# Chris10M/Lip2Speech

Hardware: AMD Instinct MI355X
Metric: mel-frames/sec at LRW batch=32, 29-frame clips (Lip2Speech.inference, S=300) (higher is better)
Workload: dtype f32; 1 GPU; LRW single-word, batch=32 per step, 29x96x96 RGB mouth crops, S=300 decode steps, speaker embedding supplied (encoding=voice), random-init weights; every step is one full pass over one B=32 batch; frames=29, decode_steps=300, library=libl2s_hip.so, parallelism=dp1 (clip sharding, no collective), batches_per_launch_chain=8, launch_chains_in_flight_per_gpu=3, distinct_batches_per_gpu=24, ranks=1

## Files before the change

### lip2speech_amd/csrc/encoder_kernels.hip

```cpp
#include "l2s_common.h"
#include <type_traits>

namespace l2s {

constexpr int FE_PR = 6;
constexpr int FE_CR = 2 * FE_PR + 1;
constexpr int FE_XROWS = 2 * (FE_CR - 1) + 7 + 1;
constexpr int FE_XLD = 104;
constexpr int FE_KP = 50;
constexpr int FE_CO = 24;

template <int HW, int MODE>
__global__ __launch_bounds__(256, 3) void frontend3d_kernel(const FrontendW w, const FrameSrc vsrc,
                                                            int T, float* __restrict__ out, float* __restrict__ zout) {
    constexpr bool SAVE_Z = MODE == 1;
    constexpr int H = HW, W = HW, Hc = H / 2, Wc = W / 2, Hp = Hc / 2, Wp = Wc / 2;
    constexpr int P = FE_CR * Wc;
    constexpr int NT = (P + 31) / 32;
    constexpr int TPW = (NT + 3) / 4;
    constexpr int XS = FE_XROWS * FE_XLD;
    constexpr int WS = FE_KP * 32;
    constexpr int CS = MODE == 2 ? 0 : P * (FE_CO / 2);
    constexpr int SMEM = (XS + WS) > CS ? (XS + WS) : CS;
    __shared__ __attribute__((aligned(16))) float smem[SMEM];
// ... 44 lines not shown
#pragma unroll
        for (int s = 0; s < FE_KP / 2; ++s) {
            const int k0 = 2 * s, k1 = 2 * s + 1;
            const int off0 = (k0 / 7) * FE_XLD + (k0 % 7);
            const int off1 = (k1 / 7) * FE_XLD + (k1 % 7);
            const int off = lg ? off1 : off0;
            const float bw = Ws[(2 * s + lg) * 32 + li];
#pragma unroll
            for (int j = 0; j < TPW; ++j) {
                if (wave + 4 * j < NT) {
                    const float a = Xs[base[j] + off];
                    acc[j] = __builtin_amdgcn_mfma_f32_32x32x2f32(a, bw, acc[j], 0, 0, 0);
                }
            }
        }
    }
    __syncthreads();

    if (MODE == 2) {
        float s1 = 0.f, s2 = 0.f;
#pragma unroll
        for (int j = 0; j < TPW; ++j) {
            if (wave + 4 * j < NT) {
#pragma unroll
                for (int r = 0; r < 16; ++r) {
                    const int p = (wave + 4 * j) * 32 + (r & 3) + 8 * (r >> 2) + 4 * lg;
                    const int lr = p / Wc, crow = 2 * p0 - 1 + lr;
                    if (p < P && lr >= 1 && crow < Hc) {
                        s1 += acc[j][r]; s2 = fmaf(acc[j][r], acc[j][r], s2);
                        if (out && li < FE_CO) out[(((int64_t)f * Hc + crow) * Wc + (p - lr * Wc)) * FE_CO + li] = acc[j][r];
                    }
                }
            }
        }
        float* red = smem;
        red[((0 * 4 + wave) * 2 + lg) * 32 + li] = s1;
        red[((1 * 4 + wave) * 2 + lg) * 32 + li] = s2;
        __syncthreads();
        if (tid < 2 * FE_CO) {
            const int k = tid / FE_CO, ch = tid - k * FE_CO;
            float t = 0.f;
            for (int q = 0; q < 8; ++q) t += red[(k * 8 + q) * 32 + ch];
            zout[((int64_t)(blockIdx.y * gridDim.x + blockIdx.x) * 2 + k) * FE_CO + ch] = t;
        }
        return;
    }
    float* Cs = smem;
    constexpr int CH = FE_CO / 2;
    const float sc = li < FE_CO ? w.scale[li] : 0.f, sh = li < FE_CO ? w.shift[li] : 0.f, sl = li < FE_CO ? w.slope[li] : 0.f;
#pragma unroll
    for (int half = 0; half < 2; ++half) {
        if (li >= half * CH && li < (half + 1) * CH) {
#pragma unroll
            for (int j = 0; j < TPW; ++j) {
                if (wave + 4 * j < NT) {
#pragma unroll
                    for (int r = 0; r < 16; ++r) {
                        const int p = (wave + 4 * j) * 32 + (r & 3) + 8 * (r >> 2) + 4 * lg;
                        if (p < P) {
                            float v = acc[j][r] * sc + sh;
                            if (SAVE_Z) {
                                const int lr = p / Wc, crow = 2 * p0 - 1 + lr;
                                if (lr >= 1 && crow < Hc) zout[(((int64_t)f * Hc + crow) * Wc + (p - lr * Wc)) * FE_CO + li] = v;
                            }
                            v = v >= 0.f ? v : sl * v;
                            Cs[p * CH + (li - half * CH)] = v;
                        }
                    }
                }
            }
        }
        __syncthreads();
        for (int i = tid; i < FE_PR * Wp * CH; i += 256) {
            const int ch = i % CH;
            const int pw = (i / CH) % Wp;
            const int prl = i / (CH * Wp);
            const int pr = p0 + prl;
            if (pr >= Hp) continue;
            float m = -INFINITY;
#pragma unroll
            for (int dr = 0; dr < 3; ++dr) {
                const int crow = 2 * pr - 1 + dr;
                if (crow < 0 || crow >= Hc) continue;
                const int lrow = 2 * prl + dr;
#pragma unroll
                for (int dc = -1; dc <= 1; ++dc) {
                    const int cc = 2 * pw + dc;
                    if (cc < 0 || cc >= Wc) continue;
                    m = fmaxf(m, Cs[(lrow * Wc + cc) * CH + ch]);
                }
            }
            out[(((int64_t)f * Hp + pr) * Wp + pw) * FE_CO + half * CH + ch] = m;
        }
        __syncthreads();
    }
}

template <int HW> struct FxGeom { static constexpr int XLD = HW == 96 ? 112 : 108, PLANE = FE_XROWS * XLD * 2; };
constexpr int FX_WROW = 48;

typedef __bf16 fx_bf16x8 __attribute__((ext_vector_type(8)));

__device__ __forceinline__ void fx_split4(const float4& v, uint2& hi, uint2& mid, uint2& lo) {
    const float f[4] = {v.x, v.y, v.z, v.w};
    unsigned h[4], m[4], l[4];
#pragma unroll
    for (int e = 0; e < 4; ++e) {
        const unsigned xb = __float_as_uint(f[e]);
        const float r1 = f[e] - __uint_as_float(xb & 0xFFFF0000u);
        const float r2 = r1 - __uint_as_float(__float_as_uint(r1) & 0xFFFF0000u);
        h[e] = xb; m[e] = __float_as_uint(r1); l[e] = __float_as_uint(r2);
    }
    hi = make_uint2(__builtin_amdgcn_perm(h[1], h[0], 0x07060302u), __builtin_amdgcn_perm(h[3], h[2], 0x07060302u));
    mid = make_uint2(__builtin_amdgcn_perm(m[1], m[0], 0x07060302u), __builtin_amdgcn_perm(m[3], m[2], 0x07060302u));
    lo = make_uint2(__builtin_amdgcn_perm(l[1], l[0], 0x07060302u), __builtin_amdgcn_perm(l[3], l[2], 0x07060302u));
}

typedef __bf16 fx_bf16x2 __attribute__((ext_vector_type(2)));
__device__ __forceinline__ unsigned fx_rne2(float a, float b) { fx_bf16x2 v = {(__bf16)a, (__bf16)b}; return __builtin_bit_cast(unsigned, v); }

template <int HW, int TERMS>
__global__ __launch_bounds__(256, 3) void frontend3d_x3_kernel(const FrontendW w, const FrameSrc vsrc, int T, float* __restrict__ out) {
    constexpr int FX_WSLAB = 4 * TERMS * 32 * FX_WROW;
    constexpr int H = HW, W = HW, Hc = H / 2, Wc = W / 2, Hp = Hc / 2, Wp = Wc / 2;
    constexpr int P = FE_CR * Wc;
    constexpr int NT = (P + 31) / 32;
    constexpr int TPW = (NT + 3) / 4;
    constexpr int XLD = FxGeom<HW>::XLD, PLANE = FxGeom<HW>::PLANE;
    static_assert((2 * (XLD / 2)) % 32 == Wc % 32 && XLD >= W + 8, "row pitch: conflict-free straddling tiles");
    constexpr int XS = TERMS * PLANE;
    constexpr int CS = P * (FE_CO / 2) * 4;
    constexpr int SMEM = (XS + FX_WSLAB) > CS ? (XS + FX_WSLAB) : CS;
    constexpr int NLD = ((FE_XROWS - 1) * (W / 4) + 255) / 256;
    constexpr int NWL = (FX_WSLAB / 16 + 255) / 256;
    __shared__ __attribute__((aligned(16))) unsigned char smem[SMEM];
    unsigned char* const Xs = smem;
    unsigned char* const Ws = smem + XS;

    const int f = blockIdx.y;
    const int bg = f / T, t = f - bg * T;
    const int grp = bg / vsrc.per, b = bg - grp * vsrc.per;
    const float* __restrict__ video = vsrc.p[grp];
    const int p0 = blockIdx.x * FE_PR;
    const int tid = threadIdx.x, wave = tid >> 6, lane = tid & 63;
    const int li = lane & 31, lg = lane >> 5;

    for (int i = tid; i < XS / 16; i += 256) reinterpret_cast<uint4*>(Xs)[i] = make_uint4(0u, 0u, 0u, 0u);

    int base[TPW];
#pragma unroll
    for (int j = 0; j < TPW; ++j) {
        int p = (wave + 4 * j) * 32 + li;
        p = p < P ? p : P - 1;
        const int lr = p / Wc, c = p - lr * Wc;
        base[j] = ((2 * lr + lg) * XLD + 2 * c) * 2;
    }
    f32x16 acc[TPW];
#pragma unroll
    for (int j = 0; j < TPW; ++j)
#pragma unroll
        for (int r = 0; r < 16; ++r) acc[j][r] = 0.f;

    const int gy0 = 4 * p0 - 5;
    auto valid = [&](int slab) { const int tt = t + (slab % 5) - 2; return tt >= 0 && tt < T; };
    auto next_valid = [&](int slab) { while (slab < 15 && !valid(slab)) ++slab; return slab; };

    float4 rin[NLD];
    uint4 rw[NWL];
    auto fetch = [&](int slab) {
        const int ci = slab / 5, kt = slab - ci * 5;
        const float* src = video + ((int64_t)(b * 3 + ci) * T + (t + kt - 2)) * (H * W);
#pragma unroll
        for (int q = 0; q < NLD; ++q) {
            const int i = tid + 256 * q;
            const int row = i / (W / 4), x4 = i - row * (W / 4);
            const int gy = gy0 + row;
            rin[q] = make_float4(0.f, 0.f, 0.f, 0.f);
            if (i < (FE_XROWS - 1) * (W / 4) && gy >= 0 && gy < H) rin[q] = *reinterpret_cast<const float4*>(src + gy * W + 4 * x4);
        }
        const uint4* wsrc = reinterpret_cast<const uint4*>(TERMS == 3 ? w.w3 : w.w1) + (int64_t)slab * (FX_WSLAB / 16);
#pragma unroll
        for (int q = 0; q < NWL; ++q) {
            const int i = tid + 256 * q;
            rw[q] = i < FX_WSLAB / 16 ? wsrc[i] : make_uint4(0u, 0u, 0u, 0u);
        }
    };
    auto stage = [&]() {
#pragma unroll
        for (int q = 0; q < NLD; ++q) {
            const int i = tid + 256 * q;
            if (i < (FE_XROWS - 1) * (W / 4)) {
                const int row = i / (W / 4), x4 = i - row * (W / 4);
                unsigned char* d = Xs + (row * XLD + 4 + 4 * x4) * 2;
                if constexpr (TERMS == 3) {
                    uint2 hi, mid, lo;
                    fx_split4(rin[q], hi, mid, lo);
                    *reinterpret_cast<uint2*>(d) = hi; *reinterpret_cast<uint2*>(d + PLANE) = mid; *reinterpret_cast<uint2*>(d + 2 * PLANE) = lo;
                } else {
                    *reinterpret_cast<uint2*>(d) = make_uint2(fx_rne2(rin[q].x, rin[q].y), fx_rne2(rin[q].z, rin[q].w));
                }
            }
        }
#pragma unroll
        for (int q = 0; q < NWL; ++q) {
            const int i = tid + 256 * q;
            if (i < FX_WSLAB / 16) reinterpret_cast<uint4*>(Ws)[i] = rw[q];
        }
    };

    int slab = next_valid(0);
    if (slab < 15) fetch(slab);
    while (slab < 15) {
        __syncthreads();
        stage();
        const int nxt = next_valid(slab + 1);
        if (nxt < 15) fetch(nxt);
        __syncthreads();
#pragma unroll
        for (int s = 0; s < 4; ++s) {
            const unsigned char* wp = Ws + ((s * TERMS) * 32 + li) * FX_WROW + lg * 16;
            const fx_bf16x8 bh = *reinterpret_cast<const fx_bf16x8*>(wp);
            if constexpr (TERMS == 1) {
#pragma unroll
                for (int j = 0; j < TPW; ++j) {
                    if (wave + 4 * j < NT) {
                        const unsigned* ap = reinterpret_cast<const unsigned*>(Xs + base[j] + s * (2 * XLD * 2));
                        const fx_bf16x8 ah = __builtin_bit_cast(fx_bf16x8, make_uint4(ap[0], ap[1], ap[2], ap[3]));
                        acc[j] = __builtin_amdgcn_mfma_f32_32x32x16_bf16(ah, bh, acc[j], 0, 0, 0);
                    }
                }
            } else {
            const fx_bf16x8 bm = *reinterpret_cast<const fx_bf16x8*>(wp + 32 * FX_WROW);
            const fx_bf16x8 bl = *reinterpret_cast<const fx_bf16x8*>(wp + 64 * FX_WROW);
#pragma unroll
            for (int j = 0; j < TPW; ++j) {
                if (wave + 4 * j < NT) {
                    const unsigned* ap = reinterpret_cast<const unsigned*>(Xs + base[j] + s * (2 * XLD * 2));
                    const unsigned* am_ = reinterpret_cast<const unsigned*>(Xs + base[j] + s * (2 * XLD * 2) + PLANE);
                    const unsigned* al_ = reinterpret_cast<const unsigned*>(Xs + base[j] + s * (2 * XLD * 2) + 2 * PLANE);
                    const fx_bf16x8 ah = __builtin_bit_cast(fx_bf16x8, make_uint4(ap[0], ap[1], ap[2], ap[3]));
                    const fx_bf16x8 am = __builtin_bit_cast(fx_bf16x8, make_uint4(am_[0], am_[1], am_[2], am_[3]));
                    const fx_bf16x8 al = __builtin_bit_cast(fx_bf16x8, make_uint4(al_[0], al_[1], al_[2], al_[3]));
                    acc[j] = __builtin_amdgcn_mfma_f32_32x32x16_bf16(al, bh, acc[j], 0, 0, 0);
                    acc[j] = __builtin_amdgcn_mfma_f32_32x32x16_bf16(ah, bl, acc[j], 0, 0, 0);
                    acc[j] = __builtin_amdgcn_mfma_f32_32x32x16_bf16(am, bm, acc[j], 0, 0, 0);
                    acc[j] = __builtin_amdgcn_mfma_f32_32x32x16_bf16(am, bh, acc[j], 0, 0, 0);
                    acc[j] = __builtin_amdgcn_mfma_f32_32x32x16_bf16(ah, bm, acc[j], 0, 0, 0);
                    acc[j] = __builtin_amdgcn_mfma_f32_32x32x16_bf16(ah, bh, acc[j], 0, 0, 0);
                }
            }
            }
        }
        slab = nxt;
    }
    __syncthreads();

    float* Cs = reinterpret_cast<float*>(smem);
    constexpr int CH = FE_CO / 2;
    const float sc = li < FE_CO ? w.scale[li] : 0.f, sh = li < FE_CO ? w.shift[li] : 0.f, sl = li < FE_CO ? w.slope[li] : 0.f;
#pragma unroll
    for (int half = 0; half < 2; ++half) {
        if (li >= half * CH && li < (half + 1) * CH) {
#pragma unroll
            for (int j = 0; j < TPW; ++j) {
                if (wave + 4 * j < NT) {
#pragma unroll
                    for (int r = 0; r < 16; ++r) {
                        const int p = (wave + 4 * j) * 32 + (r & 3) + 8 * (r >> 2) + 4 * lg;
                        if (p < P) {
                            float v = acc[j][r] * sc + sh;
                            v = v >= 0.f ? v : sl * v;
                            Cs[p * CH + (li - half * CH)] = v;
                        }
                    }
                }
            }
        }
        __syncthreads();
        for (int i = tid; i < FE_PR * Wp * CH; i += 256) {
            const int ch = i % CH;
            const int pw = (i / CH) % Wp;
            const int prl = i / (CH * Wp);
            const int pr = p0 + prl;
            if (pr >= Hp) continue;
            float m = -INFINITY;
#pragma unroll
            for (int dr = 0; dr < 3; ++dr) {
                const int crow = 2 * pr - 1 + dr;
                if (crow < 0 || crow >= Hc) continue;
                const int lrow = 2 * prl + dr;
#pragma unroll
                for (int dc = -1; dc <= 1; ++dc) {
                    const int cc = 2 * pw + dc;
                    if (cc < 0 || cc >= Wc) continue;
                    m = fmaxf(m, Cs[(lrow * Wc + cc) * CH + ch]);
                }
            }
            out[(((int64_t)f * Hp + pr) * Wp + pw) * FE_CO + half * CH + ch] = m;
        }
        __syncthreads();
    }
}

template <int HW>
__global__ __launch_bounds__(256, 2) void frontend3d_x3p_kernel(const FrontendW w, const FrameSrc vsrc, int T, float* __restrict__ out) {
    constexpr int H = HW, W = HW, Hc = H / 2, Wc = W / 2, Hp = Hc / 2, Wp = Wc / 2;
    constexpr int P = FE_CR * Wc;
    constexpr int PT = (P + 15) / 16;
    constexpr int TPW = (PT + 3) / 4;
    constexpr int XLD = 112, PLANE = FE_XROWS * XLD * 2;
    static_assert(XLD >= W + 8 && (XLD / 2) % 32 == 24, "row pitch");
    constexpr int XS = 3 * PLANE;
    constexpr int WROW = 48, LROW = 32;
    constexpr int WSP = 24 * LROW;
    constexpr int WSO = 12 * WSP;
    constexpr int WS = 2 * WSO;
    constexpr int CS = P * (FE_CO / 2) * 4;
    constexpr int SMEM = (XS + 2 * WS) > CS ? (XS + 2 * WS) : CS;
    constexpr int NLD = ((FE_XROWS - 1) * (W / 4) + 255) / 256;
    constexpr int NWU = WS / 16, NWC = NWU / 64;
    static_assert(NWU % 64 == 0, "the weight operand is a whole number of wave-wide 16-byte pieces");
    constexpr int SRC_SP = 32 * WROW / 16;
    __shared__ __attribute__((aligned(16))) unsigned char smem[SMEM];
    unsigned char* const Xs = smem;
    unsigned char* const Ws0 = smem + XS;

    const int NPAIR = (T + 1) / 2;
    const int bg = blockIdx.y / NPAIR, t0 = 2 * (blockIdx.y - bg * NPAIR);
    const bool has1 = t0 + 1 < T;
    const int grp = bg / vsrc.per, b = bg - grp * vsrc.per;
    const float* __restrict__ video = vsrc.p[grp];
    const int p0 = blockIdx.x * FE_PR;
    const int tid = threadIdx.x, wave = tid >> 6, lane = tid & 63;
    const int li = lane & 15, kg = lane >> 4;
    const int kr = ((kg & 1) << 1) | (kg >> 1);

    for (int i = tid; i < XS / 16; i += 256) reinterpret_cast<uint4*>(Xs)[i] = make_uint4(0u, 0u, 0u, 0u);

    int base[TPW];
#pragma unroll
    for (int j = 0; j < TPW; ++j) {
        int p = (wave + 4 * j) * 16 + li;
        p = p < P ? p : P - 1;
        const int lr = p / Wc, c = p - lr * Wc;
        base[j] = ((2 * lr + kr) * XLD + 2 * c) * 2;
    }
    int wof[3];
#pragma unroll
    for (int nt = 0; nt < 3; ++nt) {
        const int q = nt * 16 + li, o = q >= FE_CO ? 1 : 0, ch = q - FE_CO * o;
        wof[nt] = o * WSO + (kr >> 1) * (3 * WSP) + ch * LROW + (kr & 1) * 16;
    }
    f32x4 acc[TPW][3];
#pragma unroll
    for (int j = 0; j < TPW; ++j)
#pragma unroll
        for (int nt = 0; nt < 3; ++nt) acc[j][nt] = {0.f, 0.f, 0.f, 0.f};

    const int gy0 = 4 * p0 - 5;
    auto valid = [&](int sl) { const int d = sl % 6, tau = t0 - 2 + d; return tau >= 0 && tau < T && (d <= 4 || has1); };
    auto next_valid = [&](int sl) { while (sl < 18 && !valid(sl)) ++sl; return sl; };

    float4 rin[NLD];
    auto fetch_piece = [&](int sl, int q) {
        const int ci = sl / 6, d = sl - ci * 6;
        const float* src = video + ((int64_t)(b * 3 + ci) * T + (t0 - 2 + d)) * (H * W);
        const int i = tid + 256 * q;
        const int row = i / (W / 4), x4 = i - row * (W / 4);
        const int gy = gy0 + row;
        rin[q] = make_float4(0.f, 0.f, 0.f, 0.f);
        if (i < (FE_XROWS - 1) * (W / 4) && gy >= 0 && gy < H) rin[q] = *reinterpret_cast<const float4*>(src + gy * W + 4 * x4);
    };
    auto fetch = [&](int sl) {
#pragma unroll
        for (int q = 0; q < NLD; ++q) fetch_piece(sl, q);
    };
    auto dma_piece = [&](int sl, int buf, int kp) {
        const int c = wave + 4 * kp;
        if (c < NWC) {
            const int ci = sl / 6, d = sl - ci * 6;
            const uint4* w3 = reinterpret_cast<const uint4*>(w.w3);
            unsigned char* const Wd = Ws0 + buf * WS;
            const int i = c * 64 + lane;
            const int o = i >= NWU / 2 ? 1 : 0, r = i - o * (NWU / 2);
            const int sp = r / (WSP / 16), u = r - sp * (WSP / 16);
            const int kt = d - o;
            const bool on = kt >= 0 && kt <= 4 && (o == 0 || has1);
            const uint4* src = on ? w3 + (int64_t)(ci * 5 + kt) * (12 * SRC_SP) + sp * SRC_SP + (u >> 1) * (WROW / 16) + (u & 1) : w3 + (24 * WROW) / 16;
            __builtin_amdgcn_global_load_lds((const __attribute__((address_space(1))) void*)src,
                                             (__attribute__((address_space(3))) void*)(Wd + c * 1024), 16, 0, 0);
        }
    };
    constexpr int NDP = (NWC + 3) / 4;
    auto dma_weights = [&](int sl, int buf) {
#pragma unroll
        for (int kp = 0; kp < NDP; ++kp) dma_piece(sl, buf, kp);
    };
    auto stage = [&]() {
#pragma unroll
        for (int q = 0; q < NLD; ++q) {
            const int i = tid + 256 * q;
            if (i < (FE_XROWS - 1) * (W / 4)) {
                const int row = i / (W / 4), x4 = i - row * (W / 4);
                unsigned char* dd = Xs + (row * XLD + 4 + 4 * x4) * 2;
                uint2 hi, mid, lo;
                fx_split4(rin[q], hi, mid, lo);
                *reinterpret_cast<uint2*>(dd) = hi; *reinterpret_cast<uint2*>(dd + PLANE) = mid; *reinterpret_cast<uint2*>(dd + 2 * PLANE) = lo;
            }
        }
    };

    int sl = next_valid(0), nslab = 0;
    if (sl < 18) { fetch(sl); dma_weights(sl, 0); }
    while (sl < 18) {
        __syncthreads();
        stage();
        const int d = sl % 6;
        const bool on0 = d <= 4, on1 = d >= 1 && has1;
        const int nxt = next_valid(sl + 1);
        __syncthreads();
        const bool more = nxt < 18;
        static_assert(NDP + NLD <= 2 * TPW, "one request per pixel tile");
        const unsigned char* const Ws = Ws0 + (nslab & 1) * WS;
#pragma unroll
        for (int S = 0; S < 2; ++S) {
            fx_bf16x8 bh[3], bm[3], bl[3];
#pragma unroll
            for (int nt = 0; nt < 3; ++nt) {
                const unsigned char* wp = Ws + wof[nt] + S * (2 * 3 * WSP);
                bh[nt] = *reinterpret_cast<const fx_bf16x8*>(wp);
                bm[nt] = *reinterpret_cast<const fx_bf16x8*>(wp + WSP);
                bl[nt] = *reinterpret_cast<const fx_bf16x8*>(wp + 2 * WSP);
            }
#pragma unroll
            for (int j = 0; j < TPW; ++j) {
                if (more) {
                    const int pos = S * TPW + j;
                    if (pos < NDP) dma_piece(nxt, (nslab + 1) & 1, pos);
                    else if (pos < NDP + NLD) fetch_piece(nxt, pos - NDP);
                }
                {
                    const unsigned* ap = reinterpret_cast<const unsigned*>(Xs + base[j] + S * (4 * XLD * 2));
                    const unsigned* am_ = reinterpret_cast<const unsigned*>(Xs + base[j] + S * (4 * XLD * 2) + PLANE);
                    const unsigned* al_ = reinterpret_cast<const unsigned*>(Xs + base[j] + S * (4 * XLD * 2) + 2 * PLANE);
                    const fx_bf16x8 ah = __builtin_bit_cast(fx_bf16x8, make_uint4(ap[0], ap[1], ap[2], ap[3]));
                    const fx_bf16x8 am = __builtin_bit_cast(fx_bf16x8, make_uint4(am_[0], am_[1], am_[2], am_[3]));
                    const fx_bf16x8 al = __builtin_bit_cast(fx_bf16x8, make_uint4(al_[0], al_[1], al_[2], al_[3]));
#pragma unroll
                    for (int nt = 0; nt < 3; ++nt) {
                        if ((nt == 0 && !on0) || (nt == 2 && !on1)) continue;
                        f32x4 a = acc[j][nt];
                        a = __builtin_amdgcn_mfma_f32_16x16x32_bf16(al, bh[nt], a, 0, 0, 0);
                        a = __builtin_amdgcn_mfma_f32_16x16x32_bf16(ah, bl[nt], a, 0, 0, 0);
                        a = __builtin_amdgcn_mfma_f32_16x16x32_bf16(am, bm[nt], a, 0, 0, 0);
                        a = __builtin_amdgcn_mfma_f32_16x16x32_bf16(am, bh[nt], a, 0, 0, 0);
                        a = __builtin_amdgcn_mfma_f32_16x16x32_bf16(ah, bm[nt], a, 0, 0, 0);
                        a = __builtin_amdgcn_mfma_f32_16x16x32_bf16(ah, bh[nt], a, 0, 0, 0);
                        acc[j][nt] = a;
                    }
                }
            }
        }
        sl = nxt; ++nslab;
    }
    __syncthreads();

    float* Cs = reinterpret_cast<float*>(smem);
    constexpr int CH = FE_CO / 2;
    float sc[3], sh[3], slp[3];
#pragma unroll
    for (int nt = 0; nt < 3; ++nt) {
        const int q = nt * 16 + li, ch = q >= FE_CO ? q - FE_CO : q;
        sc[nt] = w.scale[ch]; sh[nt] = w.shift[ch]; slp[nt] = w.slope[ch];
    }
    for (int pass = 0; pass < (has1 ? 4 : 2); ++pass) {
        const int o = pass >> 1, half = pass & 1;
#pragma unroll
        for (int nt = 0; nt < 3; ++nt) {
            const int q = nt * 16 + li, qo = q >= FE_CO ? 1 : 0, ch = q - FE_CO * qo;
            if (qo == o && ch >= half * CH && ch < (half + 1) * CH) {
#pragma unroll
                for (int j = 0; j < TPW; ++j) {
                    if (wave + 4 * j < PT) {
#pragma unroll
                        for (int r = 0; r < 4; ++r) {
                            const int p = (wave + 4 * j) * 16 + 4 * kg + r;
                            if (p < P) {
                                float v = acc[j][nt][r] * sc[nt] + sh[nt];
                                v = v >= 0.f ? v : slp[nt] * v;
                                Cs[p * CH + (ch - half * CH)] = v;
                            }
                        }
                    }
                }
            }
        }
        __syncthreads();
        const int f = bg * T + t0 + o;
        for (int i = tid; i < FE_PR * Wp * CH; i += 256) {
            const int ch = i % CH;
            const int pw = (i / CH) % Wp;
            const int prl = i / (CH * Wp);
            const int pr = p0 + prl;
            if (pr >= Hp) continue;
            float m = -INFINITY;
#pragma unroll
            for (int dr = 0; dr < 3; ++dr) {
                const int crow = 2 * pr - 1 + dr;
                if (crow < 0 || crow >= Hc) continue;
                const int lrow = 2 * prl + dr;
#pragma unroll
                for (int dc = -1; dc <= 1; ++dc) {
                    const int cc = 2 * pw + dc;
                    if (cc < 0 || cc >= Wc) continue;
                    m = fmaxf(m, Cs[(lrow * Wc + cc) * CH + ch]);
                }
            }
            out[(((int64_t)f * Hp + pr) * Wp + pw) * FE_CO + half * CH + ch] = m;
        }
        __syncthreads();
    }
}

template <int HW>
__global__ __launch_bounds__(256, 2) void frontend3d_x3q_kernel(const FrontendW w, const FrameSrc vsrc, int T, float* __restrict__ out) {
    const int NPAIR = (T + 1) / 2;
    const int bg = blockIdx.y / NPAIR, t0 = 2 * (blockIdx.y - bg * NPAIR);
    const bool has1 = t0 + 1 < T;
    const int grp = bg / vsrc.per, b = bg - grp * vsrc.per;
    const float* __restrict__ video = vsrc.p[grp];
#define FE_X3Q_PITCH T
#define FE_X3Q_FRAME0 (bg * T)
#include "frontend_x3q_block.inc"
#undef FE_X3Q_PITCH
#undef FE_X3Q_FRAME0
}

template <int HW>
__global__ __launch_bounds__(256, 2) void frontend3d_x3q_ragged_kernel(const FrontendW w, const FrameSrc vsrc, const RaggedClip* __restrict__ clips,
                                                                       const int* __restrict__ pair_clip, float* __restrict__ out) {
    const RaggedClip k = clips[pair_clip[blockIdx.y]];
    const int T = k.len;
    const int t0 = 2 * ((int)blockIdx.y - k.pair0);
    const bool has1 = t0 + 1 < T;
    const int b = k.row;
    const float* __restrict__ video = vsrc.p[0];
#pragma unroll
    for (int g = 1; g < MAX_GROUP; ++g) video = k.g == g ? vsrc.p[g] : video;
#define FE_X3Q_PITCH k.T
#define FE_X3Q_FRAME0 k.frame0
#include "frontend_x3q_block.inc"
#undef FE_X3Q_PITCH
#undef FE_X3Q_FRAME0
}

int launch_frontend(const FrontendW& w, const FrameSrc& video, int B, int T, int H, int W, float* out, hipStream_t s, float* zout) {
    L2S_REQUIRE(H == W && (H == 96 || H == 88), "frontend supports 96x96 and 88x88 mouth crops");
    L2S_REQUIRE(video.per >= 1 && (B + video.per - 1) / video.per <= MAX_GROUP, "too many frame tensors in one launch");
    for (int g = 0; g < (B + video.per - 1) / video.per; ++g)
        L2S_REQUIRE(video.p[g] && (reinterpret_cast<uintptr_t>(video.p[g]) & 15u) == 0, "video must be non-null and 16-byte aligned");
    const int Hp = H / 4;
    dim3 grid((Hp + FE_PR - 1) / FE_PR, B * T);
    ProfScope ps("frontend3d_conv_bn_prelu_pool", s);
    if (!zout && w.w1) {
        if (H == 96) hipLaunchKernelGGL((frontend3d_x3_kernel<96, 1>), grid, dim3(256), 0, s, w, video, T, out);
        else hipLaunchKernelGGL((frontend3d_x3_kernel<88, 1>), grid, dim3(256), 0, s, w, video, T, out);
    } else if (!zout && w.w3 && w.pair) {
        dim3 gp((Hp + FE_PR - 1) / FE_PR, B * ((T + 1) / 2));
        if (w.pipe) {
            const unsigned pad = w.solo ? 4096u : 0u;
            if (H == 96) hipLaunchKernelGGL((frontend3d_x3q_kernel<96>), gp, dim3(256), pad, s, w, video, T, out);
            else hipLaunchKernelGGL((frontend3d_x3q_kernel<88>), gp, dim3(256), pad, s, w, video, T, out);
        } else if (H == 96) hipLaunchKernelGGL((frontend3d_x3p_kernel<96>), gp, dim3(256), 0, s, w, video, T, out);
        else hipLaunchKernelGGL((frontend3d_x3p_kernel<88>), gp, dim3(256), 0, s, w, video, T, out);
    } else if (!zout && w.w3) {
        if (H == 96) hipLaunchKernelGGL((frontend3d_x3_kernel<96, 3>), grid, dim3(256), 0, s, w, video, T, out);
        else hipLaunchKernelGGL((frontend3d_x3_kernel<88, 3>), grid, dim3(256), 0, s, w, video, T, out);
    } else if (zout) {
        if (H == 96) hipLaunchKernelGGL((frontend3d_kernel<96, 1>), grid, dim3(256), 0, s, w, video, T, out, zout);
        else hipLaunchKernelGGL((frontend3d_kernel<88, 1>), grid, dim3(256), 0, s, w, video, T, out, zout);
    } else {
        if (H == 96) hipLaunchKernelGGL((frontend3d_kernel<96, 0>), grid, dim3(256), 0, s, w, video, T, out, zout);
        else hipLaunchKernelGGL((frontend3d_kernel<88, 0>), grid, dim3(256), 0, s, w, video, T, out, zout);
    }
    L2S_CHECK_HIP(hipGetLastError());
    return 0;
}

int launch_frontend_ragged(const FrontendW& w, const FrameSrc& video, const RaggedTab& rg, int H, int W, float* out, hipStream_t s) {
    L2S_REQUIRE(H == W && (H == 96 || H == 88), "frontend supports 96x96 and 88x88 mouth crops");
    L2S_REQUIRE(w.w3 && !w.w1 && w.pair && w.pipe && !w.solo, "the ragged front-end exists in the default form only (frontend_x3 = 3, no infer_bf16)");
    L2S_REQUIRE(rg.clips && rg.pair_clip && rg.NP >= 1 && rg.NF >= 1, "ragged front-end: empty table");
    const int Hp = H / 4;
    dim3 gp((Hp + FE_PR - 1) / FE_PR, rg.NP);
    prof_count("frontend3d_ragged_pair_blocks", rg.NP);
    ProfScope ps("frontend3d_conv_bn_prelu_pool_ragged", s);
    if (H == 96) hipLaunchKernelGGL((frontend3d_x3q_ragged_kernel<96>), gp, dim3(256), 0, s, w, video, rg.clips, rg.pair_clip, out);
    else hipLaunchKernelGGL((frontend3d_x3q_ragged_kernel<88>), gp, dim3(256), 0, s, w, video, rg.clips, rg.pair_clip, out);
    L2S_CHECK_HIP(hipGetLastError());
    return 0;
}

__global__ __launch_bounds__(256) void frontend_pool_kernel(const float* __restrict__ z, const float* __restrict__ slope, int NF, int Hc, int Wc, float* __restrict__ out) {
    const int Hp = Hc / 2, Wp = Wc / 2;
    const unsigned total = (unsigned)NF * Hp * Wp * FE_CO;
    for (unsigned idx = blockIdx.x * 256u + threadIdx.x; idx < total; idx += gridDim.x * 256u) {
        const int ch = idx % FE_CO;
        unsigned r = idx / FE_CO;
        const int pw = r % Wp; r /= Wp;
        const int pr = r % Hp;
        const unsigned f = r / Hp;
        const float sl = slope[ch];
        float m = -INFINITY;
#pragma unroll
        for (int dr = -1; dr <= 1; ++dr) {
            const int crow = 2 * pr + dr;
            if (crow < 0 || crow >= Hc) continue;
#pragma unroll
            for (int dc = -1; dc <= 1; ++dc) {
                const int cc = 2 * pw + dc;
                if (cc < 0 || cc >= Wc) continue;
                float v = z[((size_t)(f * Hc + crow) * Wc + cc) * FE_CO + ch];
                v = v >= 0.f ? v : sl * v;
                m = fmaxf(m, v);
            }
        }
        out[idx] = m;
    }
}
int launch_frontend_pool(const float* z, const float* slope, int NF, int Hc, int Wc, float* out, hipStream_t s) {
    const int64_t total = (int64_t)NF * (Hc / 2) * (Wc / 2) * FE_CO;
    L2S_REQUIRE(total < (int64_t)1 << 31, "front-end pool: map too large for 32-bit indexing");
    ProfScope ps("train_frontend_prelu_pool", s);
    hipLaunchKernelGGL(frontend_pool_kernel, dim3((unsigned)std::min<int64_t>((total + 255) / 256, 16384)), dim3(256), 0, s, z, slope, NF, Hc, Wc, out);
    L2S_CHECK_HIP(hipGetLastError());
    return 0;
}

int launch_frontend_stats(const FrontendW& w, const float* video1, int B, int T, int H, int W, float* partials, int* nblocks, hipStream_t s, float* raw_out) {
    L2S_REQUIRE(H == W && (H == 96 || H == 88), "frontend supports 96x96 and 88x88 mouth crops");
    FrameSrc video{}; video.p[0] = video1; video.per = B;
    const int Hp = H / 4;
    dim3 grid((Hp + FE_PR - 1) / FE_PR, B * T);
    *nblocks = (int)(grid.x * grid.y);
    ProfScope ps("train_frontend3d_stats", s);
    if (H == 96) hipLaunchKernelGGL((frontend3d_kernel<96, 2>), grid, dim3(256), 0, s, w, video, T, raw_out, partials);
    else hipLaunchKernelGGL((frontend3d_kernel<88, 2>), grid, dim3(256), 0, s, w, video, T, raw_out, partials);
    L2S_CHECK_HIP(hipGetLastError());
    return 0;
}

struct ClipTab { int64_t off[MAX_COLLATE_CLIPS]; int frames[MAX_COLLATE_CLIPS]; };

__global__ __launch_bounds__(256) void normalise_pad_kernel(const uint8_t* __restrict__ packed, const ClipTab tab, int b0, int T, int HW4,
                                                            float* __restrict__ video) {
    const int q = blockIdx.x * 256 + threadIdx.x, t = blockIdx.y, bl = blockIdx.z;
    if (q >= HW4) return;
    const int b = b0 + bl;
    const int64_t plane = (int64_t)HW4 * 4;
    float* out = video + (((int64_t)b * 3) * T + t) * plane + (int64_t)q * 4;
    float4 r = make_float4(0.f, 0.f, 0.f, 0.f), g = r, bl4 = r;
    if (t < tab.frames[bl]) {
        const uint32_t* src = reinterpret_cast<const uint32_t*>(packed + tab.off[bl] + ((int64_t)t * plane + (int64_t)q * 4) * 3);
        const uint32_t w0 = src[0], w1 = src[1], w2 = src[2];
        const float mean[3] = {0.485f, 0.456f, 0.406f}, stdv[3] = {0.229f, 0.224f, 0.225f};
        auto nrm = [&](uint32_t byte, int c) { return __fdiv_rn(__fsub_rn(__fdiv_rn((float)byte, 255.0f), mean[c]), stdv[c]); };
        r = make_float4(nrm(w0 & 255u, 0), nrm(w0 >> 24, 0), nrm((w1 >> 16) & 255u, 0), nrm((w2 >> 8) & 255u, 0));
        g = make_float4(nrm((w0 >> 8) & 255u, 1), nrm(w1 & 255u, 1), nrm(w1 >> 24, 1), nrm((w2 >> 16) & 255u, 1));
        bl4 = make_float4(nrm((w0 >> 16) & 255u, 2), nrm((w1 >> 8) & 255u, 2), nrm(w2 & 255u, 2), nrm(w2 >> 24, 2));
    }
    *reinterpret_cast<float4*>(out) = r;
    *reinterpret_cast<float4*>(out + (int64_t)T * plane) = g;
    *reinterpret_cast<float4*>(out + 2 * (int64_t)T * plane) = bl4;
}

int launch_normalise_pad(const uint8_t* packed, const int64_t* offsets, const int* frames, int B, int T, int H, int W, float* video, hipStream_t s) {
    L2S_REQUIRE((H * W) % 4 == 0 && (reinterpret_cast<uintptr_t>(packed) & 3u) == 0 && (reinterpret_cast<uintptr_t>(video) & 15u) == 0,
                "frames: H*W must be a multiple of 4, buffers aligned");
    const int HW4 = H * W / 4;
    ProfScope ps("normalise_pad_frames", s);
    for (int b0 = 0; b0 < B; b0 += MAX_COLLATE_CLIPS) {
        const int nb = B - b0 < MAX_COLLATE_CLIPS ? B - b0 : MAX_COLLATE_CLIPS;
        ClipTab tab{};
        for (int i = 0; i < nb; ++i) {
            L2S_REQUIRE(frames[b0 + i] >= 0 && frames[b0 + i] <= T && offsets[b0 + i] % 4 == 0, "clip table: 0 <= frames <= T, 4-byte aligned offsets");
            tab.off[i] = offsets[b0 + i]; tab.frames[i] = frames[b0 + i];
        }
        hipLaunchKernelGGL(normalise_pad_kernel, dim3((HW4 + 255) / 256, T, nb), dim3(256), 0, s, packed, tab, b0, T, HW4, video);
    }
    L2S_CHECK_HIP(hipGetLastError());
    return 0;
}

__global__ __launch_bounds__(256) void dwconv3x3_kernel(const float* __restrict__ in, int N, int Hi, int Wi, int ldi,
                                                        int ci_off, int C, int stride, const float* __restrict__ w9,
                                                        const float* __restrict__ scale, const float* __restrict__ shift,
                                                        float* __restrict__ out, int Ho, int Wo, int ldo, int co_off) {
    const int64_t total = (int64_t)N * Ho * Wo * C;
    for (int64_t idx = (int64_t)blockIdx.x * 256 + threadIdx.x; idx < total; idx += (int64_t)gridDim.x * 256) {
        const int c = idx % C;
        int64_t r = idx / C;
        const int ow = r % Wo;
        r /= Wo;
        const int oh = r % Ho;
        const int n = r / Ho;
        float acc = 0.f;
#pragma unroll
        for (int kh = 0; kh < 3; ++kh) {
            const int ih = oh * stride + kh - 1;
            if (ih < 0 || ih >= Hi) continue;
#pragma unroll
            for (int kw = 0; kw < 3; ++kw) {
                const int iw = ow * stride + kw - 1;
                if (iw < 0 || iw >= Wi) continue;
                acc = fmaf(in[(((int64_t)n * Hi + ih) * Wi + iw) * ldi + ci_off + c], w9[(kh * 3 + kw) * C + c], acc);
            }
        }
        out[(((int64_t)n * Ho + oh) * Wo + ow) * ldo + co_off + c] = acc * scale[c] + shift[c];
    }
}

int launch_dwconv(const float* in, int N, int Hi, int Wi, int ldi, int ci_off, int C, int stride, const float* w9,
                  const float* scale, const float* shift, float* out, int ldo, int co_off, hipStream_t s) {
    const int Ho = (Hi + 2 - 3) / stride + 1, Wo = (Wi + 2 - 3) / stride + 1;
    const int64_t total = (int64_t)N * Ho * Wo * C;
    int blocks = (int)((total + 255) / 256);
    if (blocks > 8192) blocks = 8192;
    ProfScope ps("dwconv3x3_bn", s);
    hipLaunchKernelGGL(dwconv3x3_kernel, dim3(blocks), dim3(256), 0, s, in, N, Hi, Wi, ldi, ci_off, C, stride, w9, scale,
                       shift, out, Ho, Wo, ldo, co_off);
    L2S_CHECK_HIP(hipGetLastError());
    return 0;
}


__device__ __forceinline__ f32x4 su_mfma4(const float4& a, const float4& w, f32x4 acc) {
    acc = __builtin_amdgcn_mfma_f32_16x16x4f32(a.x, w.x, acc, 0, 0, 0);
    acc = __builtin_amdgcn_mfma_f32_16x16x4f32(a.y, w.y, acc, 0, 0, 0);
    acc = __builtin_amdgcn_mfma_f32_16x16x4f32(a.z, w.z, acc, 0, 0, 0);
    acc = __builtin_amdgcn_mfma_f32_16x16x4f32(a.w, w.w, acc, 0, 0, 0);
    return acc;
}

constexpr int su_pad16(int v) { return (v + 15) / 16 * 16; }
constexpr int su_group(int mt) { return (mt + (mt + 4) / 5 - 1) / ((mt + 4) / 5); }

template <int N_, int NC_, int MT_>
struct SuGemm {
    static constexpr int N = N_, NC = NC_, MT = MT_, G = su_group(MT_);
    static constexpr int NT = (N + 15) / 16, MG = (MT + G - 1) / G, ITEMS = NT * MG, IT = (ITEMS + 7) / 8;
};

template <class GM, int LDA>
__device__ __forceinline__ void su_gemm(float* __restrict__ buf, const float* __restrict__ Wf,
                                        const float* __restrict__ scale, const float* __restrict__ shift) {
    constexpr int NC = GM::NC, G = GM::G, IT = GM::IT, NT = GM::NT;
    const int lane = threadIdx.x & 63;
    const int wave = __builtin_amdgcn_readfirstlane(threadIdx.x >> 6);
    const int li = lane & 15, lg = lane >> 4;
    f32x4 acc[IT][G];
#pragma unroll
    for (int it = 0; it < IT; ++it) {
        const int item = wave + 8 * it;
#pragma unroll
        for (int j = 0; j < G; ++j) acc[it][j] = {0.f, 0.f, 0.f, 0.f};
        if (item < GM::ITEMS) {
            const int nt = item % NT, mg = item / NT;
            const int mt0 = min(mg * G, GM::MT - G);
            const float4* wb = reinterpret_cast<const float4*>(Wf) + nt * (NC * 64) + lane;
            const float* ab = buf + (mt0 * 16 + li) * LDA + 4 * lg;
            float4 b4[NC];
#pragma unroll
            for (int c = 0; c < NC; ++c) b4[c] = wb[c * 64];
#pragma unroll
            for (int c = 0; c < NC; ++c) {
#pragma unroll
                for (int j = 0; j < G; ++j) {
                    const float4 a4 = *reinterpret_cast<const float4*>(ab + j * 16 * LDA + 16 * c);
                    acc[it][j] = su_mfma4(a4, b4[c], acc[it][j]);
                }
                __builtin_amdgcn_sched_barrier(0);
            }
        }
    }
    __syncthreads();
#pragma unroll
    for (int it = 0; it < IT; ++it) {
        const int item = wave + 8 * it;
        if (item < GM::ITEMS) {
            const int nt = item % NT, mg = item / NT;
            const int mt0 = min(mg * G, GM::MT - G);
            const int n = nt * 16 + li;
            if (n < GM::N) {
                const float sc = scale[n], sh = shift[n];
#pragma unroll
                for (int j = 0; j < G; ++j) {
#pragma unroll
                    for (int r = 0; r < 4; ++r) {
                        const float v = acc[it][j][r] * sc + sh;
                        buf[((mt0 + j) * 16 + 4 * lg + r) * LDA + n] = v > 0.f ? v : 0.f;
                    }
                }
            }
        }
    }
    __syncthreads();
}

template <int H, int HALF, int F>
struct S1Geo {
    static constexpr int HH = H * H, C = 2 * HALF, KP = su_pad16(HALF), LDA = KP + 4, PX = F * HH;
    static constexpr int MT = (PX + 15) / 16, ROWS = MT * 16, PPW = (PX + 7) / 8, CIT = (C + 63) / 64, CH = (HALF + 63) / 64;
    using GM = SuGemm<HALF, KP / 16, MT>;
    static constexpr size_t SMEM = (size_t)ROWS * LDA * sizeof(float);
};

#ifdef L2S_DIAG
static unsigned long long* g_su_ts = nullptr;
static int g_su_ts_h = 0;
void shuffle_set_timeline(unsigned long long* ts, int h) { g_su_ts = ts; g_su_ts_h = h; }
#endif
#define SU_STAMP(k) do { if (TIMED && threadIdx.x == 0) ts[blockIdx.x * 10 + (k)] = wall_clock64(); } while (0)

template <int H, int HALF, int F, bool TIMED>
__global__ __launch_bounds__(512, 4) void shuffle_s1_kernel(const ShuffleS1P p, unsigned long long* __restrict__ ts) {
    using Q = S1Geo<H, HALF, F>;
    constexpr int HH = Q::HH, C = Q::C, KP = Q::KP, LDA = Q::LDA, ROWS = Q::ROWS, PPW = Q::PPW, CIT = Q::CIT;
    extern __shared__ __attribute__((aligned(16))) float su_smem[];
    const int tid = threadIdx.x, lane = tid & 63;
    const int wave = __builtin_amdgcn_readfirstlane(tid >> 6);
    SU_STAMP(0);
    const int f0 = blockIdx.x * F;
    const int Mv = min(F, p.NF - f0) * HH;
    float* buf = su_smem;
    const float* xb = p.x + (int64_t)f0 * HH * C;
    float* ob = p.out + (int64_t)f0 * HH * C;

    const __amdgpu_buffer_rsrc_t rsrc = __builtin_amdgcn_make_buffer_rsrc(const_cast<float*>(xb), 0, Mv * C * 4, 0x00020000);
    int voff[CIT];
#pragma unroll
    for (int j = 0; j < CIT; ++j) voff[j] = (lane + 64 * j < C) ? (lane + 64 * j) * 4 : 0x7ffffff0;
    float xr[PPW][CIT];
#pragma unroll
    for (int i = 0; i < PPW; ++i) {
        const int soff = (wave + 8 * i) * C * 4;
#pragma unroll
        for (int j = 0; j < CIT; ++j)
            xr[i][j] = __builtin_bit_cast(float, __builtin_amdgcn_raw_buffer_load_b32(rsrc, voff[j], soff, 0));
    }
    if (KP > HALF) {
        for (int idx = tid; idx < ROWS * (KP - HALF); idx += 512) {
            const int m = idx / (KP - HALF), k = HALF + idx - m * (KP - HALF);
            buf[m * LDA + k] = 0.f;
        }
    }
    for (int idx = tid; idx < (ROWS - Mv) * HALF; idx += 512) {
        const int m = Mv + idx / HALF, k = idx - (m - Mv) * HALF;
        buf[m * LDA + k] = 0.f;
    }
#pragma unroll
    for (int i = 0; i < PPW; ++i) {
        const int m = wave + 8 * i;
#pragma unroll
        for (int j = 0; j < CIT; ++j) {
            const int c = lane + 64 * j;
            if (m < Mv && c >= HALF && c < C) buf[m * LDA + (c - HALF)] = xr[i][j];
        }
    }
    SU_STAMP(1);
    __syncthreads();
    SU_STAMP(2);
    su_gemm<typename Q::GM, LDA>(buf, p.w1f, p.s1, p.b1);
    SU_STAMP(3);
    constexpr bool PAIRS = HALF > 64;
    constexpr int NROW = F * H, RPW = (NROW + 7) / 8;
    typedef float su_f2 __attribute__((ext_vector_type(2)));
    using DV = std::conditional_t<PAIRS, su_f2, float>;
    constexpr int DW = PAIRS ? 2 : 1;
    constexpr int CHD = (HALF + 64 * DW - 1) / (64 * DW);
    DV dv[CHD][RPW][H];
    const DV zero = DV{};
#pragma unroll
    for (int jc = 0; jc < CHD; ++jc) {
        const int c = min(DW * lane + 64 * DW * jc, HALF - DW);
        DV wk[9];
#pragma unroll
        for (int t = 0; t < 9; ++t) wk[t] = *reinterpret_cast<const DV*>(p.wd + t * HALF + c);
        const DV sd = *reinterpret_cast<const DV*>(p.sd + c), bd = *reinterpret_cast<const DV*>(p.bd + c);
#pragma unroll
        for (int r = 0; r < RPW; ++r) {
            const int R = wave + 8 * r;
            if (R * H < Mv) {
                const int y = R % H;
                const bool up = y > 0, dn = y < H - 1;
                const float* rm = buf + (R * H) * LDA + c;
                const float* ru = rm - (up ? H * LDA : 0);
                const float* rd = rm + (dn ? H * LDA : 0);
                DV wu[3], wdn[3];
#pragma unroll
// ... 1119 lines not shown
```

### lip2speech_amd/csrc/frontend_x3q_block.inc

```
    constexpr int H = HW, W = HW, Hc = H / 2, Wc = W / 2, Hp = Hc / 2, Wp = Wc / 2;
    constexpr int P = FE_CR * Wc;
    constexpr int PT = (P + 15) / 16;
    constexpr int TPW = (PT + 3) / 4;
    constexpr int XLD = 112, PLANE = FE_XROWS * XLD * 2;
    static_assert(XLD >= W + 8 && (XLD / 2) % 32 == 24, "row pitch");
    constexpr int XS = 3 * PLANE;
    constexpr int WROW = 48, LROW = 32;
    constexpr int WSP = 24 * LROW;
    constexpr int WSO = 12 * WSP;
    constexpr int WS = 2 * WSO;
    constexpr int CS = P * (FE_CO / 2) * 4;
    constexpr int SMEM = (2 * XS + 2 * WS) > CS ? (2 * XS + 2 * WS) : CS;
    constexpr int NLD = ((FE_XROWS - 1) * (W / 4) + 255) / 256;
    constexpr int NWU = WS / 16, NWC = NWU / 64;
    static_assert(NWU % 64 == 0, "the weight operand is a whole number of wave-wide 16-byte pieces");
    constexpr int SRC_SP = 32 * WROW / 16;
    __shared__ __attribute__((aligned(16))) unsigned char smem[SMEM];
    unsigned char* const Xs0 = smem;
    unsigned char* const Ws0 = smem + 2 * XS;

    const int p0 = blockIdx.x * FE_PR;
    const int tid = threadIdx.x, wave = tid >> 6, lane = tid & 63;
    const int li = lane & 15, kg = lane >> 4;
    const int kr = ((kg & 1) << 1) | (kg >> 1);

    for (int i = tid; i < 2 * XS / 16; i += 256) reinterpret_cast<uint4*>(Xs0)[i] = make_uint4(0u, 0u, 0u, 0u);

    int base[TPW];
#pragma unroll
    for (int j = 0; j < TPW; ++j) {
        int p = (wave + 4 * j) * 16 + li;
        p = p < P ? p : P - 1;
        const int lr = p / Wc, c = p - lr * Wc;
        base[j] = ((2 * lr + kr) * XLD + 2 * c) * 2;
    }
    int wof[3];
#pragma unroll
    for (int nt = 0; nt < 3; ++nt) {
        const int q = nt * 16 + li, o = q >= FE_CO ? 1 : 0, ch = q - FE_CO * o;
        wof[nt] = o * WSO + (kr >> 1) * (3 * WSP) + ch * LROW + (kr & 1) * 16;
    }
    f32x4 acc[TPW][3];
#pragma unroll
    for (int j = 0; j < TPW; ++j)
#pragma unroll
        for (int nt = 0; nt < 3; ++nt) acc[j][nt] = {0.f, 0.f, 0.f, 0.f};

    const int gy0 = 4 * p0 - 5;
    auto valid = [&](int sl) { const int d = sl % 6, tau = t0 - 2 + d; return tau >= 0 && tau < T && (d <= 4 || has1); };
    auto next_valid = [&](int sl) { while (sl < 18 && !valid(sl)) ++sl; return sl; };

    float4 rin[NLD];
    auto fetch_piece = [&](int sl, int q) {
        const int ci = sl / 6, d = sl - ci * 6;
        const float* src = video + ((int64_t)(b * 3 + ci) * FE_X3Q_PITCH + (t0 - 2 + d)) * (H * W);
        const int i = tid + 256 * q;
        const int row = i / (W / 4), x4 = i - row * (W / 4);
        const int gy = gy0 + row;
        rin[q] = make_float4(0.f, 0.f, 0.f, 0.f);
        if (i < (FE_XROWS - 1) * (W / 4) && gy >= 0 && gy < H) rin[q] = *reinterpret_cast<const float4*>(src + gy * W + 4 * x4);
    };
    auto fetch = [&](int sl) {
#pragma unroll
        for (int q = 0; q < NLD; ++q) fetch_piece(sl, q);
    };
    auto dma_piece = [&](int sl, int buf, int kp) {
        const int c = wave + 4 * kp;
        if (c < NWC) {
            const int ci = sl / 6, d = sl - ci * 6;
            const uint4* w3 = reinterpret_cast<const uint4*>(w.w3);
            unsigned char* const Wd = Ws0 + buf * WS;
            const int i = c * 64 + lane;
            const int o = i >= NWU / 2 ? 1 : 0, r = i - o * (NWU / 2);
            const int sp = r / (WSP / 16), u = r - sp * (WSP / 16);
            const int kt = d - o;
            const bool on = kt >= 0 && kt <= 4 && (o == 0 || has1);
            const uint4* src = on ? w3 + (int64_t)(ci * 5 + kt) * (12 * SRC_SP) + sp * SRC_SP + (u >> 1) * (WROW / 16) + (u & 1) : w3 + (24 * WROW) / 16;
            __builtin_amdgcn_global_load_lds((const __attribute__((address_space(1))) void*)src,
                                             (__attribute__((address_space(3))) void*)(Wd + c * 1024), 16, 0, 0);
        }
    };
    constexpr int NDP = (NWC + 3) / 4;
    auto dma_weights = [&](int sl, int buf) {
#pragma unroll
        for (int kp = 0; kp < NDP; ++kp) dma_piece(sl, buf, kp);
    };
    auto stage_piece = [&](unsigned char* Xd, int q) {
        const int i = tid + 256 * q;
        if (i < (FE_XROWS - 1) * (W / 4)) {
            const int row = i / (W / 4), x4 = i - row * (W / 4);
            unsigned char* dd = Xd + (row * XLD + 4 + 4 * x4) * 2;
            uint2 hi, mid, lo;
            fx_split4(rin[q], hi, mid, lo);
            *reinterpret_cast<uint2*>(dd) = hi; *reinterpret_cast<uint2*>(dd + PLANE) = mid; *reinterpret_cast<uint2*>(dd + 2 * PLANE) = lo;
        }
    };

    int sl = next_valid(0), nslab = 0;
    if (sl < 18) {
        fetch(sl); dma_weights(sl, 0);
        __syncthreads();
#pragma unroll
        for (int q = 0; q < NLD; ++q) stage_piece(Xs0, q);
    }
    static_assert(NLD + NDP + NLD <= 2 * TPW, "one request / one staging piece per pixel tile");
    while (sl < 18) {
        __syncthreads();
        const int d = sl % 6;
        const bool on0 = d <= 4, on1 = d >= 1 && has1;
        const int nxt = next_valid(sl + 1);
        const bool more = nxt < 18;
        const unsigned char* const Xs = Xs0 + (nslab & 1) * XS;
        unsigned char* const Xn = Xs0 + ((nslab + 1) & 1) * XS;
        const unsigned char* const Ws = Ws0 + (nslab & 1) * WS;
#pragma unroll
        for (int S = 0; S < 2; ++S) {
            fx_bf16x8 bh[3], bm[3], bl[3];
#pragma unroll
            for (int nt = 0; nt < 3; ++nt) {
                const unsigned char* wp = Ws + wof[nt] + S * (2 * 3 * WSP);
                bh[nt] = *reinterpret_cast<const fx_bf16x8*>(wp);
                bm[nt] = *reinterpret_cast<const fx_bf16x8*>(wp + WSP);
                bl[nt] = *reinterpret_cast<const fx_bf16x8*>(wp + 2 * WSP);
            }
#pragma unroll
            for (int j = 0; j < TPW; ++j) {
                if (more) {
                    const int pos = S * TPW + j;
                    if (pos < NLD) fetch_piece(nxt, pos);
                    else if (pos < NLD + NDP) dma_piece(nxt, (nslab + 1) & 1, pos - NLD);
                    else if (pos >= 2 * TPW - NLD) stage_piece(Xn, pos - (2 * TPW - NLD));
                }
                {
                    const unsigned* ap = reinterpret_cast<const unsigned*>(Xs + base[j] + S * (4 * XLD * 2));
                    const unsigned* am_ = reinterpret_cast<const unsigned*>(Xs + base[j] + S * (4 * XLD * 2) + PLANE);
                    const unsigned* al_ = reinterpret_cast<const unsigned*>(Xs + base[j] + S * (4 * XLD * 2) + 2 * PLANE);
                    const fx_bf16x8 ah = __builtin_bit_cast(fx_bf16x8, make_uint4(ap[0], ap[1], ap[2], ap[3]));
                    const fx_bf16x8 am = __builtin_bit_cast(fx_bf16x8, make_uint4(am_[0], am_[1], am_[2], am_[3]));
                    const fx_bf16x8 al = __builtin_bit_cast(fx_bf16x8, make_uint4(al_[0], al_[1], al_[2], al_[3]));
#pragma unroll
                    for (int nt = 0; nt < 3; ++nt) {
                        if ((nt == 0 && !on0) || (nt == 2 && !on1)) continue;
                        f32x4 a = acc[j][nt];
                        a = __builtin_amdgcn_mfma_f32_16x16x32_bf16(al, bh[nt], a, 0, 0, 0);
                        a = __builtin_amdgcn_mfma_f32_16x16x32_bf16(ah, bl[nt], a, 0, 0, 0);
                        a = __builtin_amdgcn_mfma_f32_16x16x32_bf16(am, bm[nt], a, 0, 0, 0);
                        a = __builtin_amdgcn_mfma_f32_16x16x32_bf16(am, bh[nt], a, 0, 0, 0);
                        a = __builtin_amdgcn_mfma_f32_16x16x32_bf16(ah, bm[nt], a, 0, 0, 0);
                        a = __builtin_amdgcn_mfma_f32_16x16x32_bf16(ah, bh[nt], a, 0, 0, 0);
                        acc[j][nt] = a;
                    }
                }
            }
        }
        sl = nxt; ++nslab;
    }
    __syncthreads();

    float* Cs = reinterpret_cast<float*>(smem);
    constexpr int CH = FE_CO / 2;
    float sc[3], sh[3], slp[3];
#pragma unroll
    for (int nt = 0; nt < 3; ++nt) {
        const int q = nt * 16 + li, ch = q >= FE_CO ? q - FE_CO : q;
        sc[nt] = w.scale[ch]; sh[nt] = w.shift[ch]; slp[nt] = w.slope[ch];
    }
    for (int pass = 0; pass < (has1 ? 4 : 2); ++pass) {
        const int o = pass >> 1, half = pass & 1;
#pragma unroll
        for (int nt = 0; nt < 3; ++nt) {
            const int q = nt * 16 + li, qo = q >= FE_CO ? 1 : 0, ch = q - FE_CO * qo;
            if (qo == o && ch >= half * CH && ch < (half + 1) * CH) {
#pragma unroll
                for (int j = 0; j < TPW; ++j) {
                    if (wave + 4 * j < PT) {
#pragma unroll
                        for (int r = 0; r < 4; ++r) {
                            const int p = (wave + 4 * j) * 16 + 4 * kg + r;
                            if (p < P) {
                                float v = acc[j][nt][r] * sc[nt] + sh[nt];
                                v = v >= 0.f ? v : slp[nt] * v;
                                Cs[p * CH + (ch - half * CH)] = v;
                            }
                        }
                    }
                }
            }
        }
        __syncthreads();
        const int f = FE_X3Q_FRAME0 + t0 + o;
        for (int i = tid; i < FE_PR * Wp * CH; i += 256) {
            const int ch = i % CH;
            const int pw = (i / CH) % Wp;
            const int prl = i / (CH * Wp);
            const int pr = p0 + prl;
            if (pr >= Hp) continue;
            float m = -INFINITY;
#pragma unroll
            for (int dr = 0; dr < 3; ++dr) {
                const int crow = 2 * pr - 1 + dr;
                if (crow < 0 || crow >= Hc) continue;
                const int lrow = 2 * prl + dr;
#pragma unroll
                for (int dc = -1; dc <= 1; ++dc) {
                    const int cc = 2 * pw + dc;
                    if (cc < 0 || cc >= Wc) continue;
                    m = fmaxf(m, Cs[(lrow * Wc + cc) * CH + ch]);
                }
            }
            out[(((int64_t)f * Hp + pr) * Wp + pw) * FE_CO + half * CH + ch] = m;
        }
        __syncthreads();
    }
```

### lip2speech_amd/csrc/l2s_common.h

```cpp
#pragma once
#include <hip/hip_runtime.h>
#include <stdint.h>
#include <string>

#define L2S_WAVE 64

typedef float f32x4 __attribute__((ext_vector_type(4)));
typedef float f32x16 __attribute__((ext_vector_type(16)));

namespace l2s {

void set_error(const std::string& msg);
#define L2S_CHECK_HIP(expr)                                                                   \
    do {                                                                                      \
        hipError_t _e = (expr);                                                               \
        if (_e != hipSuccess) {                                                               \
            l2s::set_error(std::string(#expr) + ": " + hipGetErrorString(_e));                \
            return 1;                                                                         \
        }                                                                                     \
    } while (0)
#define L2S_REQUIRE(cond, msg)                                                                \
    do {                                                                                      \
        if (!(cond)) {                                                                        \
            l2s::set_error(std::string("l2s: ") + (msg) + " [" #cond "]");                    \
            return 1;                                                                         \
        }                                                                                     \
    } while (0)

void prof_begin(const char* name, hipStream_t s);
void prof_end(hipStream_t s);
void prof_count(const char* name, int64_t n);
struct ProfScope {
    hipStream_t s;
    ProfScope(const char* name, hipStream_t st) : s(st) { prof_begin(name, st); }
    ~ProfScope() { prof_end(s); }
};

struct Options {
    int fold = 1;
    int graph = 0;
    int overlap_postnet = 0;
    int fuse_trunk = 1;
    int fuse_s2 = 1;
    int trunk_x3 = 1;
    int refresh_map = 0;
    int skinny_static = 0;
    int skinny_sized = 1;
    int skinny_split = 2;
    int skinny_split8 = 1;
    int rc_shape = 0;
    int rc_jb = 0;
    int gemm_x3_dma = 1;
    int lstm_x3 = 4;
    int half_min_mts = 12;
    int flat_half = 1;
    int attn_lds = 1;
    int hoist_vproj = 2;
    int skinny_flat = 1;
    int rc_shape_multi = 0;
    int gemm_x3 = 1;
    int frontend_x3 = 3;
    int train_bf16 = 0;
    int persist = 4;
    int persist_frames = 32;
    int persist_masked = 0;
    int frontend_solo = 0;
    int trunk_chain = 1;
    int flat_xcd = 1;
    int attn_skip0 = 1;
    int early_stop = 0;
    int infer_bf16 = 0;
};
int set_option_field(Options& o, const char* name, int value);

enum Act { ACT_NONE = 0, ACT_RELU = 1, ACT_SILU = 2, ACT_PSINE = 3, ACT_PRELU = 4  };

struct GemmP {
    const float* A;
    const float* W;
    const float* scale;
    const float* shift;
    const float* actw;
    const float* R1;
    const float* R2;
    float* C;
    int M, N, K;
    int lda, Tout, Tin, taps, stride, pad, Cin;
    int a_split, a_gap;
    int act;
    int ldr1, r1_mod, ldr2, r2_mod;
    int r2_div;
    int ldc, c_cstride;
    int c_tr_T;
    float* Zout;
    int win_T, win_off;
    int vec;
    const float* mask;
    int ldmask, mask_pre;
    int ldw;
    const void* W3;
    int x3;
    int x3_group;
    float* stats;
    int stats_raw;
};
inline int64_t gemm_stats_floats(int M, int N) { return (int64_t)((M + 63) / 64) * 2 * N; }
constexpr int GEMM_MAX_GROUP = 8;
struct GemmBatch {
    GemmP p[GEMM_MAX_GROUP];
    int count;
};
GemmP gemm_plain(const float* A, int lda, const float* W, float* C, int ldc, int M, int N, int K);
int& gemm_x3_mode();
int& gemm_x3_group();
struct X3Scope { int prev; explicit X3Scope(int on) : prev(gemm_x3_mode()) { gemm_x3_mode() = on; } ~X3Scope() { gemm_x3_mode() = prev; } };
int& chains_hint();
bool& grouped_entry();
struct X3Group {
    int prev; bool prev_grouped;
    explicit X3Group(int g) : prev(gemm_x3_group()), prev_grouped(grouped_entry()) { gemm_x3_group() = g; grouped_entry() = true; }
    ~X3Group() { gemm_x3_group() = prev; grouped_entry() = prev_grouped; }
};
int& gemm_bf16_mode();
struct Bf16Scope { int prev; explicit Bf16Scope(int on) : prev(gemm_bf16_mode()) { gemm_bf16_mode() = on; } ~Bf16Scope() { gemm_bf16_mode() = prev; } };
bool gemm_x3_eligible(const GemmBatch& b);
bool gemm_x3_member_ok(const GemmP& p);
int64_t gemm_planes_bytes(int N, int K);
int launch_gemm_planes(const float* W, int N, int K, void* planes, hipStream_t s);
int launch_gemm_x3(const GemmBatch& b, hipStream_t s, const char* name);
void gemm_x3_set_timeline(unsigned long long* ts, int block);
int launch_gemm_splitk(const GemmP& p, int ksplit, float* part, hipStream_t s, const char* name);
int launch_gemm_splitk_group(const GemmBatch& g, int ksplit, float* part, hipStream_t s, const char* name);
int launch_gemm_tapsplit(const GemmBatch& convs, float* part, hipStream_t s, const char* name);
int launch_gemm(const GemmBatch& b, hipStream_t s, const char* name);
int launch_gemm_finish(const GemmBatch& b, hipStream_t s, const char* name);
int launch_gemm1(const GemmP& p, hipStream_t s, const char* name);

enum BwdMode { BWD_DX = 0, BWD_DW = 1 };
struct BwdGemmP {
    int mode;
    const float* A; int lda;
    const float* B; int ldb;
    float* C; int ldc;
    int M, N, K;
    int Tx, Tz, taps, stride, pad, padp, Nout, Cin;
    int c_T; int64_t c_seq_stride;
    float alpha; int accumulate;
    int vec;
    int ksplit; int64_t c_split_stride;
};
BwdGemmP bwd_dx(const float* dZ, int ldz, const float* Wp, float* dX, int ldx, int B, int Tz, int Tx, int Nout, int Cin, int taps, int pad, bool accumulate);
BwdGemmP bwd_dw(const float* dZ, int ldz, const float* X, int ldx, float* dWp, int B, int Tz, int Tx, int Nout, int Cin, int taps, int stride, int pad, bool accumulate);
int launch_gemm_bwd(const BwdGemmP& p, hipStream_t s, const char* name);
int64_t gemm_bwd_splitk_floats(const BwdGemmP& p, int splits);
int launch_gemm_bwd_splitk(const BwdGemmP& p, int splits, float* partials, hipStream_t s, const char* name);
int launch_gemm_bwd_dw_dx(const BwdGemmP& pdw, int splits, float* partials, const BwdGemmP& pdx, hipStream_t s, const char* name);

constexpr int AB_RS = 1024;
struct ActBwdP {
    const float* dy; const float* z; float* dconv;
    int ld_dy, ld_z, ld_dconv;
    int64_t rows; int C;
    int act;
    const float* actw;
    const float* scale;
    const float* gamma; const float* beta;
    float* partials;
    int cs_dy, co_dy, cs_z, co_z;
};
int act_bwd(const ActBwdP& p, float* d_shift, float* d_gamma, float* d_actw, float* d_convbias, bool accumulate, hipStream_t s, float* totals = nullptr);

struct BnLayer {
    const float* gamma; const float* beta; float* rmean; float* rvar; const float* conv_bias;
    float* scale; float* shift;
    int C;
};
int bn_stats_finalize(const float* partials, int nblk, int blk_stride, int64_t count, const BnLayer& L, float momentum, hipStream_t s);
int bn_train_fix(float* dconv, int ld_dconv, const float* z, int ld_z, int cs_z, int co_z, const float* gamma, const float* beta, const float* scale,
                 const float* totals, int64_t rows, int C, hipStream_t s);
constexpr int DWS_RS = 1024;
int launch_dwconv_stats(const float* in, int N, int Hi, int Wi, int ldi, int ci_off, int C, int stride, const float* w9, float* partials, hipStream_t s,
                        float* raw_out = nullptr, int ldo = 0, int co_off = 0);
int launch_bn_apply(float* x, int64_t rows, int C, int ld, int co_off, const float* scale, const float* shift, hipStream_t s, bool fused = false);

struct FrontendW {
    const float* w;
    const float* scale;
    const float* shift;
    const float* slope;
    const float* w3;
    int pair = 0;
    int solo = 0;
    int pipe = 0;
    const float* w1;
};
constexpr int MAX_GROUP = 8;
struct FrameSrc { const float* p[MAX_GROUP]; int per; };
int launch_frontend(const FrontendW& w, const FrameSrc& video, int B, int T, int H, int W, float* out, hipStream_t s, float* zout = nullptr);
inline int launch_frontend(const FrontendW& w, const float* video, int B, int T, int H, int W, float* out, hipStream_t s, float* zout = nullptr) {
    FrameSrc f{}; f.p[0] = video; f.per = B;
    return launch_frontend(w, f, B, T, H, W, out, s, zout);
}
struct RaggedClip { int g, row, T, len, frame0, pair0; };
constexpr int RAGGED_CHUNK = 32;
struct RaggedChunk { RaggedClip c[RAGGED_CHUNK]; int n; };
struct RaggedTab { const RaggedClip* clips; const int* pair_clip; int N, Tmax, NF, NP; };
int launch_ragged_table(const RaggedClip* clips_host, int N, RaggedClip* clips_dev, int* pair_clip_dev, hipStream_t s);
int launch_frontend_ragged(const FrontendW& w, const FrameSrc& video, const RaggedTab& rg, int H, int W, float* out, hipStream_t s);
struct EvalClip { int S, T, row, mT, mel_off, stop_off, attn_off, dis_off; };
constexpr int EVAL_CHUNK = 32;
struct EvalChunk { EvalClip c[EVAL_CHUNK]; int n; };
struct EvalTab { const EvalClip* clips; int N, Smax, Tmax, mTmax; };
enum EvalField { EV_STOP = 0, EV_ATTN = 1, EV_DIS = 2, EV_MEL_POST = 3 };
int launch_eval_table(const EvalClip* clips_host, int N, EvalClip* clips_dev, hipStream_t s);
int launch_zero_rows_past_s(float* x, int cols, const EvalTab& ev, hipStream_t s);
int launch_eval_scatter(int field, const float* src, const EvalTab& ev, float* dst, hipStream_t s);
int launch_eval_mel_cf(const float* mel, const EvalTab& ev, float* mel_cf, hipStream_t s);
int launch_frontend_stats(const FrontendW& w, const float* video, int B, int T, int H, int W, float* partials , int* nblocks, hipStream_t s, float* raw_out = nullptr);
int launch_frontend_pool(const float* z, const float* slope, int NF, int Hc, int Wc, float* out, hipStream_t s);

constexpr int MAX_COLLATE_CLIPS = 64;
int launch_normalise_pad(const uint8_t* packed, const int64_t* offsets, const int* frames, int B, int T, int H, int W, float* video, hipStream_t s);
int launch_dwconv(const float* in, int N, int Hi, int Wi, int ldi, int ci_off, int C, int stride,
                  const float* w9 , const float* scale, const float* shift,
                  float* out, int ldo, int co_off, hipStream_t s);
struct ShuffleS1P {
    const float* x; float* out;
    const float* w1f; const float* s1; const float* b1;
    const float* wd; const float* sd; const float* bd;
    const float* w2f; const float* s2; const float* b2;
    int NF, h, half, Kpad, F;
    const void* w1p; const void* w2p;
};
int64_t su_planes_bytes(int N, int K);
int launch_su_planes(const float* W, int N, int K, void* out, hipStream_t s);
int launch_shuffle_s1(const ShuffleS1P& p, hipStream_t s);
constexpr int S1_CHAIN_MAX = 7;
int launch_shuffle_s1_chain(const ShuffleS1P* units, int n, hipStream_t s);
void shuffle_set_timeline(unsigned long long* ts, int h);
struct ShuffleS2P {
    const float* x; float* out;
    const float* wd1; const float* sd1; const float* bd1;
    const float* wb1f; const float* sb1; const float* bb1;
    const float* w1f; const float* s1; const float* b1;
    const float* wd; const float* sd; const float* bd;
    const float* w2f; const float* s2; const float* b2;
    int NF, h, ho, cin, half, Kin, Kh, Ro;
    const void* wb1p; const void* w1p; const void* w2p;
};
int launch_shuffle_s2(const ShuffleS2P& p, hipStream_t s);
int launch_copy_cols(const float* in, int ldi, int off_i, float* out, int ldo, int off_o, int cs_o,
                     int64_t rows, int cols, hipStream_t s);
int launch_pool_norm_cat(const float* x, int NF, int P, int C, const float* emb, int E, int T,
                         float* vis, int ldv, float* feat , hipStream_t s);
int launch_pool_norm_cat_ragged(const float* x, const RaggedTab& rg, int P, int C, const float* emb, int E, float* vis, int ldv, hipStream_t s);

__host__ __device__ inline int64_t frag16_index(int row, int k, int K) {
    int rt = row >> 4, i = row & 15, c = k >> 4, g = (k >> 2) & 3, e = k & 3;
    return ((int64_t)(rt * (K >> 4) + c) * 64 + (g * 16 + i)) * 4 + e;
}

enum SkinnyEpi {
    SK_PLAIN = 0,
    SK_FRAG = 1,
    SK_LSTM = 2,
    SK_MEL = 3,
};
struct SkinnySeg { const float* a; int nchunks; };
struct SkinnyP {
    SkinnySeg seg[4];
    int nseg;
    const float* a_sum;
    int layout;
    const float* W;
    const void* W3;
    const float* bias;
    const float* actw;
    const float* add;
    int ld_add;
    const float* addrow;
    float* out;
    int ldo;
    int B, N, K;
    int act;
    int epi;
    const float* pre;
    int64_t ld_pre;
    const float* c_in;
    float* c_out;
    float* h_out;
    int h_out_K, h_out_off;
    float* h_seq;
    int64_t ld_hseq;
    float* h_plain;
    int ld_hplain;
    int H;
    float* mel; int64_t ld_mel_b;
    float* stop; int64_t ld_stop_b;
    const float* stop_const;
    float* yfrag;
    int* es_ctl; int es_end;
};
struct EsCtl { int end_rel; int count; int crossed[1]; };
constexpr int ES_POST_LAYERS = 5, ES_POST_TAPS = 5;
constexpr int ES_MARGIN = ES_POST_LAYERS * (ES_POST_TAPS / 2);
constexpr int SKINNY_MAX_GROUP = 4;
struct SkinnyBatch { SkinnyP p[SKINNY_MAX_GROUP]; int ntiles[SKINNY_MAX_GROUP]; int count; const int* es_end; int es_step; };
#define L2S_ES_RETURN(arg) do { if ((arg).es_end && (arg).es_step >= *(arg).es_end) return; } while (0)
int launch_skinny(const SkinnyBatch& b, hipStream_t s, const char* name, const Options& o = Options());
int launch_skx_planes(const float* Wf, int ntiles, int K, void* out, hipStream_t s);
bool skinny_sum_supported(const Options& o);
void attn_set_timeline(unsigned long long* ts);
void skinny_set_flat_timeline(unsigned long long* ts);
void skinny_set_timeline(unsigned long long* ts);

int launch_probe(int kind, int blocks, int n_per_block, const float* in, float* out, hipStream_t s);
void skinny_set_flat_timeline(unsigned long long* ts);
int set_stamp_log(unsigned long long* log, long long cap);
const void* skinny_form_kernel(const SkinnyBatch& bl, const Options& o, int chains, bool stamped_skinny, bool stamped_flat, dim3& grid, int& block, int& lds);

struct AttnP {
    const float* q; int ldq;
    const float* k;
    const float* v;
    const float* vp;
    const float* tau;
    float* av_frag;
    float* attn_out; int64_t ld_attn_b; int attn_logits;
    const float* qc; int ldqc;
    const float* ckey;
    const float* cval;
    const float* tau_c;
    float* cc_frag;
    int B, T, m;
    const int* es_end; int es_step;
};
int launch_step_attn(const AttnP& at, const SkinnyP& pre2, int pre2_tiles, hipStream_t s, int lds_values = 1, int skip0 = 0);
struct PoolCatP { const float* x[5]; int L[5]; int ld[5]; int nmaps; int B, m, C; float* out; };
int launch_pool_cat(const PoolCatP& p, hipStream_t s);
int launch_gumbel_softmax(const float* logits, const float* gumbel, int rows, int n, float tau,
                          float* z, int ldz, float* dis, hipStream_t s);
int launch_to_frag(const float* x, int ldx, int B, int K, float* frag, int Kfrag, int koff, int broadcast_row, hipStream_t s);
int launch_fill(float* p, int64_t n, float v, hipStream_t s);
int launch_from_frag(const float* frag, int Kfrag, int B, int K, float* out, int ldo, int ooff, hipStream_t s);
int launch_tile_rows(const float* src, int lds, float* dst, int ldd, int B, int T, int C, hipStream_t s);
int launch_transpose_bsc(const float* in, int B, int S, int C, float* out, hipStream_t s);
int launch_output_lengths(const float* stop, int B, int S, int64_t* lengths, hipStream_t s);
int launch_mask_by_lengths(const int64_t* lengths, int B, int S, int T, float* mel_post, float* attn, hipStream_t s);
constexpr int LEN_CHUNK = 64;
struct LenChunk { int len[LEN_CHUNK]; int n; };
int launch_len_table(const int32_t* lens_host, int B, int* table, hipStream_t s);
int launch_bilstm_capture(const float* h_frag, const float* c_frag, const int* lens, int B, int t, float* h_dst_frag, float* c_dst, int ld_c, hipStream_t s);
int launch_bilstm_reset(float* h_frag, float* c_frag, const int* lens, int B, int t, const float* s_e, hipStream_t s);
int launch_mask_copy_rows(float* x, int ldx, float* out, int ldo, const int* lens, int B, int T, int cols, hipStream_t s);
struct PoolDiv { int div[5]; };
int launch_pool_cat_masked(const PoolCatP& p, const PoolDiv& d, const int* lens, hipStream_t s);
int launch_zero_slot_rows(float* z, int ldz, float* dis, int n, int B, int m, const int* lens, hipStream_t s);
int launch_step_attn_masked(const AttnP& at, const SkinnyP& pre2, int pre2_tiles, const int* lens, hipStream_t s, int lds_values = 1, int skip0 = 0);
int launch_frame_window(const float* audio, int B, int N, int L, int n_fft, int hop, const float* window, float* frames, hipStream_t s);
int launch_power(const float* spec, int lds, int64_t rows, int nf, float* power, int ldp, hipStream_t s);
struct SpkRank { int64_t off; int32_t n; int32_t b; };
constexpr int SPK_CHUNK = 512;
struct SpkChunk { int32_t v[SPK_CHUNK]; int n; };
int launch_spk_table(const int32_t* words_host, int64_t n_words, int32_t* table, hipStream_t s);
int launch_frame_window_packed(const float* audio_packed, const SpkRank* ranks, const int* step_row0, int B, int L_max, int n_fft, int hop, const float* window,
                               float* frames, hipStream_t s);
int launch_spk_last_hidden(const float* hseq, const SpkRank* ranks, const int* step_row0, int B, float* h_last, hipStream_t s);
constexpr int IM_MAXF = 576;
constexpr int IM_MAXM = 128;
constexpr int IM_NNZ = 2048;
int launch_mel_bands(const float* fb, int n_freqs, int n_mels, int* tab, float* fwd, float* bwd, hipStream_t s);
int launch_stop_const(const float* ecell, const float* w_tail, const float* bias, int B, float* out, hipStream_t s);

}
```

### lip2speech_amd/csrc/l2s_pack.hip

```cpp
#include "l2s_common.h"
#include "l2s_model.h"

#include <algorithm>
#include <cmath>
#include <cstring>
#include <string>
#include <unordered_map>
#include <vector>

namespace l2s {

__host__ __device__ inline void bn_fold(float g, float beta, float mu, float var, float bias, float eps, float* scale, float* shift) {
#ifdef __HIP_DEVICE_COMPILE__
    const float root = __fsqrt_rn(var + eps);
#else
    const float root = std::sqrt(var + eps);
#endif
    const float s = g / root;
    *scale = s;
    *shift = (bias - mu) * s + beta;
}

struct FePlaneElem { uint16_t split[3], rne; };
__host__ __device__ inline FePlaneElem fe_plane_elem(const float* w, int slab, int st, int n, int k) {
    const int kh = 2 * st + (k >> 3), kw = (k & 7) - 1, ci = slab / 5, kt = slab % 5;
    float x = 0.f;
    if (n < 24 && kh < 7 && kw >= 0) x = w[(((int64_t)n * 3 + ci) * 5 + kt) * 49 + kh * 7 + kw];
    const uint32_t xb = __builtin_bit_cast(uint32_t, x), hb = xb & 0xFFFF0000u;
    const float r1 = x - __builtin_bit_cast(float, hb);
    const uint32_t mb = __builtin_bit_cast(uint32_t, r1) & 0xFFFF0000u;
    const float r2 = r1 - __builtin_bit_cast(float, mb);
    const uint32_t lb = __builtin_bit_cast(uint32_t, r2);
    return {{(uint16_t)(hb >> 16), (uint16_t)(mb >> 16), (uint16_t)(lb >> 16)}, (uint16_t)((xb + 0x7FFFu + ((xb >> 16) & 1u)) >> 16)};
}
constexpr int FE_W3_SLAB = 9216, FE_W1_SLAB = 3072, FE_PLANE_ELEMS = 15 * 4 * 32 * 16;
__host__ __device__ inline void fe_plane_store(const FePlaneElem& e, int slab, int st, int n, int k, uint16_t* w3, uint16_t* w1) {
    for (int pl = 0; pl < 3; ++pl) w3[(int64_t)slab * FE_W3_SLAB + ((st * 3 + pl) * 32 + n) * 24 + k] = e.split[pl];
    w1[(int64_t)slab * FE_W1_SLAB + (st * 32 + n) * 24 + k] = e.rne;
}
__host__ __device__ inline void fe_plane_fill(const float* w, int idx, uint16_t* w3, uint16_t* w1) {
    const int k = idx & 15, n = (idx >> 4) & 31, st = (idx >> 9) & 3, slab = idx >> 11;
    fe_plane_store(fe_plane_elem(w, slab, st, n, k), slab, st, n, k, w3, w1);
}

struct Blob {
    std::vector<float> data;
    int64_t alloc(int64_t n) {
        int64_t off = align_up((int64_t)data.size(), 64);
        data.resize(off + n, 0.f);
        return off;
    }
};

struct Parts { bool enc = false, dec = false, spk = false, face = false; };

struct Packer {
    l2s_model* m;
    Blob blob;
    Parts parts;
    std::vector<std::pair<const float**, int64_t>> fixups;
    std::string missing;

    const std::vector<float>* get(const std::string& key, int64_t numel) {
        auto it = m->host.find(key);
        if (it == m->host.end()) { if (missing.empty()) missing = "missing tensor " + key; return nullptr; }
        if ((int64_t)it->second.size() != numel) {
            if (missing.empty()) missing = "tensor " + key + " has " + std::to_string(it->second.size()) + " elements, expected " + std::to_string(numel);
            return nullptr;
        }
        return &it->second;
    }
    void bind(const float** slot, int64_t off) { fixups.emplace_back(slot, off); }

    std::vector<l2s_model::RefreshBn> bn_rec;
    std::vector<l2s_model::RefreshSum> sum_rec;
    void fold(int64_t so, int64_t ho, int c, const std::vector<float>& g, const std::vector<float>& b, const std::vector<float>& mu, const std::vector<float>& var,
              const std::vector<float>* bias, float eps) {
        for (int i = 0; i < c; ++i) bn_fold(g[i], b[i], mu[i], var[i], bias ? (*bias)[i] : 0.f, eps, &blob.data[so + i], &blob.data[ho + i]);
    }
    void bn(const std::string& p, int c, const std::vector<float>* bias, const float** scale, const float** shift, const std::string& bias_key = std::string(),
            float eps = BN_EPS, bool record = true) {
        auto g = get(p + ".weight", c), b = get(p + ".bias", c), mu = get(p + ".running_mean", c), var = get(p + ".running_var", c);
        if (!g || !b || !mu || !var) return;
        int64_t so = blob.alloc(c), ho = blob.alloc(c);
        fold(so, ho, c, *g, *b, *mu, *var, bias, eps);
        bind(scale, so);
        bind(shift, ho);
        if (record) bn_rec.push_back({p, bias_key, c, so, ho});
    }
    void copy(const std::string& key, int64_t n, const float** slot) {
        auto v = get(key, n);
        if (!v) return;
        int64_t o = blob.alloc(n);
        std::memcpy(&blob.data[o], v->data(), n * sizeof(float));
        bind(slot, o);
    }
    void conv1d_w(const std::string& key, int co, int ci, int k, const float** slot) {
        auto v = get(key, (int64_t)co * ci * k);
        if (!v) return;
        int64_t o = blob.alloc((int64_t)co * ci * k);
        for (int n = 0; n < co; ++n)
            for (int c = 0; c < ci; ++c)
                for (int t = 0; t < k; ++t) blob.data[o + ((int64_t)n * k + t) * ci + c] = (*v)[((int64_t)n * ci + c) * k + t];
        bind(slot, o);
    }
    void dw_w(const std::string& key, int c, const float** slot) {
        auto v = get(key, (int64_t)c * 9);
        if (!v) return;
        int64_t o = blob.alloc((int64_t)c * 9);
        for (int ch = 0; ch < c; ++ch)
            for (int t = 0; t < 9; ++t) blob.data[o + (int64_t)t * c + ch] = (*v)[(int64_t)ch * 9 + t];
        bind(slot, o);
    }
    template <typename RowFn>
    void frag16(int Npad, int K, RowFn row_of, const float** slot) {
        int64_t o = blob.alloc((int64_t)Npad * K);
        const int NC = K / 16;
        std::vector<float> row(K);
        for (int n = 0; n < Npad; ++n) {
            bool nz = row_of(n, row.data());
            if (!nz) continue;
            for (int k = 0; k < K; ++k) {
                int tile = n >> 4, i = n & 15, c = k >> 4, g = (k >> 2) & 3, e = k & 3;
                blob.data[o + ((int64_t)(tile * NC + c) * 64 + g * 16 + i) * 4 + e] = row[k];
            }
        }
        bind(slot, o);
    }
};

static int lstm_perm_row(int np, int H) {
    int unit = np >> 2, gate = np & 3;
    return gate * H + unit;
}

static const std::string E = "encoder.", Dk = "decoder.", Sk = "speaker_encoder.", Fk = "vgg_face.";

static void pack_encoder(Packer& P, Weights& w) {
    {
        auto v = P.get(E + "frontend3D.0.weight", 24 * 3 * 5 * 49);
        if (v) {
            int64_t o = P.blob.alloc(15 * 50 * 32);
            for (int co = 0; co < 24; ++co)
                for (int ci = 0; ci < 3; ++ci)
                    for (int kt = 0; kt < 5; ++kt)
                        for (int tap = 0; tap < 49; ++tap)
                            P.blob.data[o + ((int64_t)(ci * 5 + kt) * 50 + tap) * 32 + co] = (*v)[(((int64_t)co * 3 + ci) * 5 + kt) * 49 + tap];
            P.bind(&w.fe.w, o);
            const int64_t o3 = P.blob.alloc(15 * FE_W3_SLAB / 2), o1 = P.blob.alloc(15 * FE_W1_SLAB / 2);
            std::vector<uint16_t> w3(15 * FE_W3_SLAB, 0), w1(15 * FE_W1_SLAB, 0);
            for (int idx = 0; idx < FE_PLANE_ELEMS; ++idx) fe_plane_fill(v->data(), idx, w3.data(), w1.data());
            std::memcpy(&P.blob.data[o3], w3.data(), w3.size() * 2);
            std::memcpy(&P.blob.data[o1], w1.data(), w1.size() * 2);
            P.bind(&w.fe.w3, o3);
            P.bind(&w.fe.w1, o1);
        }
        P.bn(E + "frontend3D.1", 24, nullptr, &w.fe.scale, &w.fe.shift);
        P.copy(E + "frontend3D.2.weight", 24, &w.fe.slope);
    }
    {
        int u = 0, cin = STAGE_CH[0];
        for (int st = 0; st < 3; ++st) {
            int cout = STAGE_CH[st + 1], half = cout / 2;
            for (int r = 0; r < STAGE_REP[st]; ++r, ++u) {
                UnitW& U = w.unit[u];
                std::string p = E + "trunk.0." + std::to_string(u) + ".";
                U.stride2 = (r == 0);
                U.cin = cin;
                U.half = half;
                int pw1_in = U.stride2 ? cin : half;
                if (U.stride2) {
                    P.dw_w(p + "banch1.0.weight", cin, &U.b1_dw.w9);
                    P.bn(p + "banch1.1", cin, nullptr, &U.b1_dw.scale, &U.b1_dw.shift);
                    P.copy(p + "banch1.2.weight", (int64_t)half * cin, &U.b1_pw.W);
                    P.bn(p + "banch1.3", half, nullptr, &U.b1_pw.scale, &U.b1_pw.shift);
                }
                P.copy(p + "banch2.0.weight", (int64_t)half * pw1_in, &U.pw1.W);
                P.bn(p + "banch2.1", half, nullptr, &U.pw1.scale, &U.pw1.shift);
                P.dw_w(p + "banch2.3.weight", half, &U.dw.w9);
                P.bn(p + "banch2.4", half, nullptr, &U.dw.scale, &U.dw.shift);
                P.copy(p + "banch2.5.weight", (int64_t)half * half, &U.pw2.W);
                P.bn(p + "banch2.6", half, nullptr, &U.pw2.scale, &U.pw2.shift);
                {
                    U.kpad = pad16(half);
                    U.kin = pad16(pw1_in);
                    struct { const char* key; int K, Kp; const float** slot; } fr[3] = {
                        {"banch2.0.weight", pw1_in, U.stride2 ? U.kin : U.kpad, &U.pw1_frag},
                        {"banch2.5.weight", half, U.kpad, &U.pw2_frag},
                        {"banch1.2.weight", cin, U.kin, &U.b1_frag}};
                    for (int which = 0; which < (U.stride2 ? 3 : 2); ++which) {
                        const int K = fr[which].K, Kp = fr[which].Kp;
                        auto wv = P.get(p + fr[which].key, (int64_t)half * K);
                        if (!wv) continue;
                        P.frag16(pad16(half), Kp, [&](int n, float* row) {
                            if (n >= half) return false;
                            std::memset(row, 0, sizeof(float) * Kp);
                            std::memcpy(row, wv->data() + (int64_t)n * K, sizeof(float) * K);
                            return true;
                        }, fr[which].slot);
                    }
                }
                cin = cout;
            }
        }
        P.copy(E + "trunk.1.0.weight", (int64_t)LAST_CH * STAGE_CH[3], &w.conv_last.W);
        P.bn(E + "trunk.1.1", LAST_CH, nullptr, &w.conv_last.scale, &w.conv_last.shift);
    }
}

static void pack_decoder(Packer& P, Weights& w) {
    auto linear = [&](const std::string& p, int co, int ci, ConvW& c) {
        P.copy(p + ".weight", (int64_t)co * ci, &c.W);
        P.copy(p + ".bias", co, &c.shift);
    };
    P.conv1d_w(Dk + "residual_bottleneck.weight", D, 1024, 1, &w.resid.W);
    P.copy(Dk + "residual_bottleneck.bias", D, &w.resid.shift);
    linear(Dk + "encoder_site.0.linear_layer", D, 256, w.enc_site);
    P.copy(Dk + "encoder_site.1.w", D, &w.enc_site.actw);
    linear(Dk + "attention_site.0.linear_layer", D, 256, w.attn_site);
    P.copy(Dk + "attention_site.1.w", D, &w.attn_site.actw);
    linear(Dk + "E_C.linear_layer", D, 1024, w.e_c);
    linear(Dk + "encoder_proj.linear_layer", D, 1024, w.enc_proj);
    {
        const char* suf[2] = {"l0", "l0_reverse"};
        int64_t wo = P.blob.alloc((int64_t)4096 * 1024), bo = P.blob.alloc(4096);
        for (int d = 0; d < 2; ++d) {
            auto wi = P.get(Dk + "encoder_rnn.weight_ih_" + suf[d], (int64_t)2048 * 1024);
            auto bi = P.get(Dk + "encoder_rnn.bias_ih_" + suf[d], 2048), bh = P.get(Dk + "encoder_rnn.bias_hh_" + suf[d], 2048);
            auto wh = P.get(Dk + "encoder_rnn.weight_hh_" + suf[d], (int64_t)2048 * 512);
            if (!wi || !bi || !bh || !wh) continue;
            std::memcpy(&P.blob.data[wo + (int64_t)d * 2048 * 1024], wi->data(), sizeof(float) * 2048 * 1024);
            for (int i = 0; i < 2048; ++i) P.blob.data[bo + d * 2048 + i] = (*bi)[i] + (*bh)[i];
            P.sum_rec.push_back({Dk + "encoder_rnn.bias_ih_" + suf[d], Dk + "encoder_rnn.bias_hh_" + suf[d], 2048, 0, bo + d * 2048});
            P.frag16(2048, 512, [&](int np, float* row) {
                std::memcpy(row, wh->data() + (int64_t)lstm_perm_row(np, 512) * 512, sizeof(float) * 512);
                return true;
            }, &w.whh[d].W);
            w.whh[d].N = 2048; w.whh[d].K = 512; w.whh[d].tiles = 128;
        }
        P.bind(&w.wih_cat, wo);
        P.bind(&w.bih_cat, bo);
    }
    for (int kv = 0; kv < 2; ++kv) {
        std::string p = Dk + (kv == 0 ? "K" : "V");
        for (int j = 0; j < 4; ++j) {
            std::string c = p + ".0.conv." + std::to_string(j);
            P.conv1d_w(c + ".0.weight", D, D, MH_KS[j], &w.mh_branch[kv][j].W);
            P.bn(c + ".1", D, P.get(c + ".0.bias", D), &w.mh_branch[kv][j].scale, &w.mh_branch[kv][j].shift, c + ".0.bias");
        }
        P.conv1d_w(p + ".0.bottleneck.weight", D, 5 * D, 1, &w.mh_bott[kv].W);
        P.copy(p + ".0.bottleneck.bias", D, &w.mh_bott[kv].shift);
        P.copy(p + ".1.w", D, &w.mh_bott[kv].actw);
    }
    P.copy(Dk + "positional_encodings.pos_table", (int64_t)L2S_MAX_STEPS * D, &w.pos);
    for (int j = 0; j < 4; ++j) {
        std::string c = Dk + "content.agg." + std::to_string(j);
        P.conv1d_w(c + ".0.weight", D, D, CT_KS[j], &w.ct_branch[j].W);
        P.bn(c + ".1", D, P.get(c + ".0.bias", D), &w.ct_branch[j].scale, &w.ct_branch[j].shift, c + ".0.bias");
    }
    P.conv1d_w(Dk + "content.bottleneck.weight", 256, 5 * D, 1, &w.ct_bott.W);
    P.copy(Dk + "content.bottleneck.bias", 256, &w.ct_bott.shift);
    linear(Dk + "content.K.0", 256, 256, w.ct_k0);
    linear(Dk + "content.K.2", 256, 256, w.ct_k2);
    linear(Dk + "content.location_fc.0", 256, 256, w.ct_fc0);
    linear(Dk + "content.location_fc.2", 256, 256, w.ct_fc2);
    linear(Dk + "content.location_fc.4", VOC, 256, w.ct_fc4);
    {
        auto v = P.get(Dk + "content.word_embeddings", (int64_t)VOC * 256);
        if (v) {
            int64_t o = P.blob.alloc((int64_t)256 * VOCP);
            for (int n = 0; n < 256; ++n)
                for (int k = 0; k < VOC; ++k) P.blob.data[o + (int64_t)n * VOCP + k] = (*v)[(int64_t)k * 256 + n];
            P.bind(&w.ct_emb.W, o);
        }
    }
    auto sk_linear = [&](const std::string& wkey, const std::string& bkey, int N, int K, SkW& s) {
        auto wv = P.get(wkey, (int64_t)N * K);
        int Np = pad16(N);
        if (wv)
            P.frag16(Np, K, [&](int n, float* row) {
                if (n >= N) return false;
                std::memcpy(row, wv->data() + (int64_t)n * K, sizeof(float) * K);
                return true;
            }, &s.W);
        auto bv = P.get(bkey, N);
        if (bv) {
            int64_t o = P.blob.alloc(Np);
            std::memcpy(&P.blob.data[o], bv->data(), sizeof(float) * N);
            P.bind(&s.bias, o);
        }
        s.N = N; s.K = K; s.tiles = Np / 16;
    };
    sk_linear(Dk + "prenet.0.linear_layer.weight", Dk + "prenet.0.linear_layer.bias", 256, NM, w.pre1);
    P.copy(Dk + "prenet.1.w", 256, &w.pre1.actw);
    sk_linear(Dk + "prenet.3.linear_layer.weight", Dk + "prenet.3.linear_layer.bias", 256, 256, w.pre2);
    P.copy(Dk + "prenet.4.w", 256, &w.pre2.actw);
    sk_linear(Dk + "Q.0.linear_layer.weight", Dk + "Q.0.linear_layer.bias", D, 1024, w.q);
    P.copy(Dk + "Q.1.w", D, &w.q.actw);
    sk_linear(Dk + "content.Q.0.weight", Dk + "content.Q.0.bias", 256, 1024, w.cq);
    sk_linear(Dk + "attention_proj.linear_layer.weight", Dk + "attention_proj.linear_layer.bias", 256, D, w.aproj);
    int64_t lstm0_bias = -1;
    for (int l = 0; l < 2; ++l) {
        SkW& s = l == 0 ? w.lstm0 : w.lstm1;
        std::string sl = "l" + std::to_string(l);
        auto wi = P.get(Dk + "decoder_rnn.weight_ih_" + sl, (int64_t)2048 * 512), wh = P.get(Dk + "decoder_rnn.weight_hh_" + sl, (int64_t)2048 * 512);
        auto bi = P.get(Dk + "decoder_rnn.bias_ih_" + sl, 2048), bh = P.get(Dk + "decoder_rnn.bias_hh_" + sl, 2048);
        if (!wi || !wh || !bi || !bh) continue;
        P.frag16(2048, 1024, [&](int np, float* row) {
            int r = lstm_perm_row(np, 512);
            std::memcpy(row, wi->data() + (int64_t)r * 512, sizeof(float) * 512);
            std::memcpy(row + 512, wh->data() + (int64_t)r * 512, sizeof(float) * 512);
            return true;
        }, &s.W);
        int64_t o = P.blob.alloc(2048);
        for (int np = 0; np < 2048; ++np) { int r = lstm_perm_row(np, 512); P.blob.data[o + np] = (*bi)[r] + (*bh)[r]; }
        P.bind(&s.bias, o);
        if (l == 0) lstm0_bias = o;
        P.sum_rec.push_back({Dk + "decoder_rnn.bias_ih_" + sl, Dk + "decoder_rnn.bias_hh_" + sl, 2048, 512, o});
        s.N = 2048; s.K = 1024; s.tiles = 128;
    }
    {
        auto wf = P.get(Dk + "fc_out.linear_layer.weight", (int64_t)NM * D), bf = P.get(Dk + "fc_out.linear_layer.bias", NM);
        auto ws = P.get(Dk + "stop_token_layer.linear_layer.weight", 1024);
        if (wf && bf && ws) {
            P.frag16(96, D, [&](int n, float* row) {
                if (n < NM) std::memcpy(row, wf->data() + (int64_t)n * D, sizeof(float) * D);
                else if (n == NM) std::memcpy(row, ws->data(), sizeof(float) * D);
                else return false;
                return true;
            }, &w.fc.W);
            int64_t o = P.blob.alloc(96);
            std::memcpy(&P.blob.data[o], bf->data(), sizeof(float) * NM);
            P.bind(&w.fc.bias, o);
            int64_t t = P.blob.alloc(D);
            std::memcpy(&P.blob.data[t], ws->data() + D, sizeof(float) * D);
            P.bind(&w.stop_tail, t);
        }
        w.fc.N = NM + 1; w.fc.K = D; w.fc.tiles = 6;
        P.copy(Dk + "stop_token_layer.linear_layer.bias", 1, &w.stop_bias);
    }
    {
        auto wp1 = P.get(Dk + "prenet.0.linear_layer.weight", (int64_t)256 * NM), bp1 = P.get(Dk + "prenet.0.linear_layer.bias", 256);
        auto wo = P.get(Dk + "fc_out.linear_layer.weight", (int64_t)NM * D), bo = P.get(Dk + "fc_out.linear_layer.bias", NM);
        if (wp1 && bp1 && wo && bo) {
            std::vector<float> wf((size_t)256 * D);
            int64_t bo_off = P.blob.alloc(256);
            std::vector<double> row(D);
            for (int n = 0; n < 256; ++n) {
                std::fill(row.begin(), row.end(), 0.0);
                double bacc = (*bp1)[n];
                for (int k = 0; k < NM; ++k) {
                    const double a = (*wp1)[(int64_t)n * NM + k];
                    const float* wr = wo->data() + (int64_t)k * D;
                    for (int j = 0; j < D; ++j) row[j] += a * wr[j];
                    bacc += a * (*bo)[k];
                }
                for (int j = 0; j < D; ++j) wf[(size_t)n * D + j] = (float)row[j];
                P.blob.data[bo_off + n] = (float)bacc;
            }
            P.frag16(256, D, [&](int n, float* r) { std::memcpy(r, wf.data() + (size_t)n * D, sizeof(float) * D); return true; }, &w.pre1f.W);
            P.bind(&w.pre1f.bias, bo_off);
            P.copy(Dk + "prenet.1.w", 256, &w.pre1f.actw);
            w.pre1f.N = 256; w.pre1f.K = D; w.pre1f.tiles = 16;
        }
        auto wi = P.get(Dk + "decoder_rnn.weight_ih_l0", (int64_t)2048 * 512), wh = P.get(Dk + "decoder_rnn.weight_hh_l0", (int64_t)2048 * 512);
        auto bi = P.get(Dk + "decoder_rnn.bias_ih_l0", 2048), bh = P.get(Dk + "decoder_rnn.bias_hh_l0", 2048);
        auto wap = P.get(Dk + "attention_proj.linear_layer.weight", (int64_t)256 * D), bap = P.get(Dk + "attention_proj.linear_layer.bias", 256);
        if (wi && wh && bi && bh && wap && bap) {
            std::vector<float> prod((size_t)2048 * D);
            std::vector<float> badd(2048);
            std::vector<double> row(D);
            for (int r = 0; r < 2048; ++r) {
                std::fill(row.begin(), row.end(), 0.0);
                double bacc = 0.0;
                for (int k = 0; k < 256; ++k) {
                    const double a = (*wi)[(int64_t)r * 512 + 256 + k];
                    const float* wr = wap->data() + (int64_t)k * D;
                    for (int j = 0; j < D; ++j) row[j] += a * wr[j];
                    bacc += a * (*bap)[k];
                }
                for (int j = 0; j < D; ++j) prod[(size_t)r * D + j] = (float)row[j];
                badd[r] = (float)((double)(*bi)[r] + (double)(*bh)[r] + bacc);
            }
            P.frag16(2048, 1536, [&](int np, float* rowp) {
                int r = lstm_perm_row(np, 512);
                std::memcpy(rowp, wi->data() + (int64_t)r * 512, sizeof(float) * 512);
                std::memcpy(rowp + 512, prod.data() + (size_t)r * D, sizeof(float) * D);
                std::memcpy(rowp + 1024, wh->data() + (int64_t)r * 512, sizeof(float) * 512);
                return true;
            }, &w.lstm0f.W);
            int64_t o = P.blob.alloc(2048);
            for (int np = 0; np < 2048; ++np) P.blob.data[o + np] = badd[lstm_perm_row(np, 512)];
            P.bind(&w.lstm0f.bias, o);
            w.lstm0f.N = 2048; w.lstm0f.K = 1536; w.lstm0f.tiles = 128;
            P.frag16(2048, 1280, [&](int np, float* rowp) {
                int r = lstm_perm_row(np, 512);
                std::memcpy(rowp, wi->data() + (int64_t)r * 512, sizeof(float) * 512);
                std::memcpy(rowp + 512, wi->data() + (int64_t)r * 512 + 256, sizeof(float) * 256);
                std::memcpy(rowp + 768, wh->data() + (int64_t)r * 512, sizeof(float) * 512);
                return true;
            }, &w.lstm0v.W);
            P.bind(&w.lstm0v.bias, lstm0_bias);
            w.lstm0v.N = 2048; w.lstm0v.K = 1280; w.lstm0v.tiles = 128;
            P.copy(Dk + "attention_proj.linear_layer.weight", (int64_t)256 * D, &w.vproj.W);
            P.copy(Dk + "attention_proj.linear_layer.bias", 256, &w.vproj.shift);
        }
    }
    P.copy(Dk + "BOS", NM, &w.bos);
    P.copy(Dk + "temperature", 1, &w.tau);
    P.copy(Dk + "content.temperature", 1, &w.tau_c);
    for (int i = 0; i < 5; ++i) {
        int ci = i == 0 ? NM : D, co = i == 4 ? NM : D;
        std::string c = Dk + "postnet.convolutions." + std::to_string(i);
        P.conv1d_w(c + ".0.conv.weight", co, ci, 5, &w.post[i].W);
        P.bn(c + ".1", co, P.get(c + ".0.conv.bias", co), &w.post[i].scale, &w.post[i].shift, c + ".0.conv.bias");
        if (i < 4) P.copy(Dk + "postnet.sin_activation." + std::to_string(i) + ".w", D, &w.post[i].actw);
    }
}

static void pack_speaker(Packer& P, Weights& w) {
    constexpr int NFFT = 400, NF = 201, NMEL = 40, NFP = 204;
    {
        const double PI = 3.14159265358979323846;
        int64_t wo = P.blob.alloc(NFFT), dof = P.blob.alloc((int64_t)2 * NF * NFFT), fo = P.blob.alloc((int64_t)NMEL * NFP);
        for (int j = 0; j < NFFT; ++j) P.blob.data[wo + j] = (float)(0.5 - 0.5 * std::cos(2.0 * PI * j / NFFT));
        for (int k = 0; k < NF; ++k)
            for (int j = 0; j < NFFT; ++j) {
                const double ang = 2.0 * PI * (double)((int64_t)k * j % NFFT) / NFFT;
                P.blob.data[dof + (int64_t)k * NFFT + j] = (float)std::cos(ang);
                P.blob.data[dof + (int64_t)(NF + k) * NFFT + j] = (float)std::sin(ang);
            }
        std::vector<double> fpts(NMEL + 2);
        const double m_min = 0.0, m_max = 2595.0 * std::log10(1.0 + 8000.0 / 700.0);
        for (int i = 0; i < NMEL + 2; ++i) {
            const double mpt = m_min + (m_max - m_min) * i / (NMEL + 1);
            fpts[i] = 700.0 * (std::pow(10.0, mpt / 2595.0) - 1.0);
        }
        for (int k = 0; k < NF; ++k) {
            const double f = 8000.0 * k / (NF - 1);
            for (int mm = 0; mm < NMEL; ++mm) {
                const double down = (f - fpts[mm]) / (fpts[mm + 1] - fpts[mm]);
                const double up = (fpts[mm + 2] - f) / (fpts[mm + 2] - fpts[mm + 1]);
                P.blob.data[fo + (int64_t)mm * NFP + k] = (float)std::max(0.0, std::min(down, up));
            }
        }
        P.bind(&w.spk_window, wo); P.bind(&w.spk_dft, dof); P.bind(&w.spk_fbT, fo);
    }
    for (int l = 0; l < 3; ++l) {
        const int in = l == 0 ? 40 : 256;
        const std::string sl = "l" + std::to_string(l);
        auto wi = P.get(Sk + "lstm.weight_ih_" + sl, (int64_t)1024 * in), wh = P.get(Sk + "lstm.weight_hh_" + sl, (int64_t)1024 * 256);
        auto bi = P.get(Sk + "lstm.bias_ih_" + sl, 1024), bh = P.get(Sk + "lstm.bias_hh_" + sl, 1024);
        if (!wi || !wh || !bi || !bh) continue;
        P.copy(Sk + "lstm.weight_ih_" + sl, (int64_t)1024 * in, &w.spk_ih[l].W);
        int64_t bo = P.blob.alloc(1024);
        for (int i = 0; i < 1024; ++i) P.blob.data[bo + i] = (*bi)[i] + (*bh)[i];
        P.bind(&w.spk_ih[l].shift, bo);
        P.frag16(1024, 256, [&](int np, float* row) {
            std::memcpy(row, wh->data() + (int64_t)lstm_perm_row(np, 256) * 256, sizeof(float) * 256);
            return true;
        }, &w.spk_hh[l].W);
        w.spk_hh[l].N = 1024; w.spk_hh[l].K = 256; w.spk_hh[l].tiles = 64;
    }
    P.copy(Sk + "linear.weight", (int64_t)256 * 256, &w.spk_linear.W);
    P.copy(Sk + "linear.bias", 256, &w.spk_linear.shift);
}

static int pack_face(Packer& P, Weights& w) {
    const auto& layers = face_layers();
    if ((int)layers.size() != FACE_N_CONVS) { set_error("l2s_model_finalize: face layer table has " + std::to_string(layers.size()) + " entries"); return 1; }
    for (int li = 0; li < FACE_N_CONVS; ++li) {
        const FaceLayer& L = layers[li];
        const int np = (int)L.parts.size(), N = L.cout * np, taps = L.kh * L.kw, K = taps * L.cin;
        const int64_t wn = (int64_t)L.cout * K;
        std::vector<const std::vector<float>*> wt(np), g(np), b(np), mu(np), var(np);
        bool ok = true;
        for (int j = 0; j < np; ++j) {
            const std::string pre = Fk + L.parts[j];
            if (L.res_scale == 0.f) {
                wt[j] = P.get(pre + ".conv.weight", wn);
                g[j] = P.get(pre + ".bn.weight", L.cout); b[j] = P.get(pre + ".bn.bias", L.cout);
                mu[j] = P.get(pre + ".bn.running_mean", L.cout); var[j] = P.get(pre + ".bn.running_var", L.cout);
                ok = ok && wt[j] && g[j] && b[j] && mu[j] && var[j];
            } else {
                wt[j] = P.get(pre + ".weight", wn); b[j] = P.get(pre + ".bias", L.cout);
                ok = ok && wt[j] && b[j];
            }
        }
        if (!ok) continue;
        const int64_t wo = P.blob.alloc((int64_t)N * K), so = P.blob.alloc(N), ho = P.blob.alloc(N);
        for (int j = 0; j < np; ++j) {
            const std::vector<float>& v = *wt[j];
            for (int n = 0; n < L.cout; ++n) {
                const int64_t row = wo + (int64_t)(j * L.cout + n) * K;
                for (int ci = 0; ci < L.cin; ++ci)
                    for (int t = 0; t < taps; ++t) P.blob.data[row + (int64_t)t * L.cin + ci] = v[((int64_t)n * L.cin + ci) * taps + t];
                if (L.res_scale != 0.f) {
                    P.blob.data[so + j * L.cout + n] = L.res_scale;
                    P.blob.data[ho + j * L.cout + n] = (*b[j])[n] * L.res_scale;
                }
            }
            if (L.res_scale == 0.f) P.fold(so + j * L.cout, ho + j * L.cout, L.cout, *g[j], *b[j], *mu[j], *var[j], nullptr, FACE_BN_EPS);
        }
        P.bind(&w.face.convs[li].w, wo); P.bind(&w.face.convs[li].scale, so); P.bind(&w.face.convs[li].shift, ho);
    }
    auto transposed = [&](const std::string& key, int out, int in, const float** slot) {
        auto v = P.get(key, (int64_t)out * in);
        if (!v) return;
        const int64_t o = P.blob.alloc((int64_t)out * in);
        for (int r = 0; r < out; ++r)
            for (int c = 0; c < in; ++c) P.blob.data[o + (int64_t)c * out + r] = (*v)[(int64_t)r * in + c];
        P.bind(slot, o);
    };
    transposed(Fk + "resnet.last_linear.weight", 512, 1792, &w.face.tail.llT);
    P.bn(Fk + "resnet.last_bn", 512, nullptr, &w.face.tail.bn_s, &w.face.tail.bn_h, std::string(), FACE_BN_EPS, false);
    transposed(Fk + "projection_layer.0.weight", 512, 512, &w.face.tail.p0T);
    P.copy(Fk + "projection_layer.0.bias", 512, &w.face.tail.p0b);
    transposed(Fk + "projection_layer.2.weight", 256, 512, &w.face.tail.p2T);
    P.copy(Fk + "projection_layer.2.bias", 256, &w.face.tail.p2b);
    return 0;
}

static int pack_host(l2s_model* m, Packer& P) {
    m->w = Weights{};
    Weights& w = m->w;
    auto has_prefix = [&](const std::string& pre) {
        for (auto& kv : m->host) if (kv.first.compare(0, pre.size(), pre) == 0) return true;
        return false;
    };
    P.parts = Parts{has_prefix(E), has_prefix(Dk), has_prefix(Sk), has_prefix(Fk)};
    if (!P.parts.enc && !P.parts.dec && !P.parts.spk && !P.parts.face) {
        set_error("l2s_model_finalize: no encoder.* / decoder.* / speaker_encoder.* / vgg_face.* tensors were set");
        return 1;
    }
    if (P.parts.enc) pack_encoder(P, w);
    if (P.parts.dec) pack_decoder(P, w);
    if (P.parts.spk) pack_speaker(P, w);
    if (P.parts.face && pack_face(P, w)) return 1;
    if (!P.missing.empty()) { set_error("l2s_model_finalize: " + P.missing); return 1; }
    return 0;
}

static int build_refresh_map(l2s_model* m, const Packer& P, hipStream_t stream);

struct PlaneItem { const float* W; int a, b; const void** slot; };
typedef int64_t (*PlaneBytesFn)(int a, int b);
typedef int (*PlaneLaunchFn)(const float* W, int a, int b, void* out, hipStream_t s);
static int derive_planes(const std::vector<PlaneItem>& items, PlaneBytesFn bytes, PlaneLaunchFn launch, void** pool, hipStream_t s) {
    int64_t total = 0;
    for (const PlaneItem& it : items) { if (!it.W) return 0; total += bytes(it.a, it.b); }
    if (!total) return 0;
    if (!*pool) L2S_CHECK_HIP(hipMalloc(pool, total));
    char* base = reinterpret_cast<char*>(*pool);
    for (const PlaneItem& it : items) {
        if (launch(it.W, it.a, it.b, base, s)) return 1;
        *it.slot = base;
        base += bytes(it.a, it.b);
    }
    return 0;
}

static int derive_lstm_planes(l2s_model* m, hipStream_t s) {
    Weights& w = m->w;
    std::vector<PlaneItem> items;
    for (SkW* k : {&w.lstm0, &w.lstm1, &w.whh[0], &w.whh[1]}) {
        k->W3 = nullptr;
        items.push_back({k->W, k->tiles, k->K, &k->W3});
    }
    if (!m->has_dec) return 0;
    for (const PlaneItem& it : items) if (it.b % 256) return 0;
    return derive_planes(items, [](int tiles, int K) { return (int64_t)tiles * K * 96; }, launch_skx_planes, &m->lstm_planes, s);
}

static int derive_gemm_planes(l2s_model* m, hipStream_t s) {
    Weights& w = m->w;
    for (int i = 0; i < 5; ++i) w.post[i].W3 = nullptr;
    w.wih_cat3 = nullptr; w.conv_last.W3 = nullptr;
    for (int kv = 0; kv < 2; ++kv) for (int j = 0; j < 4; ++j) w.mh_branch[kv][j].W3 = nullptr;
    std::vector<PlaneItem> items;
    if (m->has_dec) {
        const int Ks[4] = {5 * NM, 5 * 512, 5 * 512, 5 * 512};
        for (int i = 0; i < 4; ++i) items.push_back({w.post[i].W, 512, Ks[i], &w.post[i].W3});
        items.push_back({w.wih_cat, 4096, 1024, &w.wih_cat3});
        for (int kv = 0; kv < 2; ++kv)
            for (int j = 0; j < 4; ++j) items.push_back({w.mh_branch[kv][j].W, 512, 512 * MH_KS[j], &w.mh_branch[kv][j].W3});
    }
    if (m->has_enc) items.push_back({w.conv_last.W, LAST_CH, STAGE_CH[3], &w.conv_last.W3});
    return derive_planes(items, gemm_planes_bytes, launch_gemm_planes, &m->gemm_planes, s);
}

static int derive_unit_planes(l2s_model* m, hipStream_t s) {
    std::vector<PlaneItem> items;
    for (UnitW& U : m->w.unit) {
        U.pw1_p3 = nullptr; U.pw2_p3 = nullptr; U.b1_p3 = nullptr;
        items.push_back({U.pw1.W, U.half, U.stride2 ? U.cin : U.half, &U.pw1_p3});
        items.push_back({U.pw2.W, U.half, U.half, &U.pw2_p3});
        if (U.stride2) items.push_back({U.b1_pw.W, U.half, U.cin, &U.b1_p3});
    }
    if (!m->has_enc) return 0;
    return derive_planes(items, su_planes_bytes, launch_su_planes, &m->unit_planes, s);
}

static int derive_all_planes(l2s_model* m, hipStream_t s, bool fresh) {
    struct { void** pool; int (*derive)(l2s_model*, hipStream_t); } kinds[3] = {
        {&m->lstm_planes, derive_lstm_planes}, {&m->gemm_planes, derive_gemm_planes}, {&m->unit_planes, derive_unit_planes}};
    for (auto& k : kinds) {
        if (fresh && *k.pool) { (void)hipFree(*k.pool); *k.pool = nullptr; }
        if ((fresh || *k.pool) && k.derive(m, s)) return 1;
    }
    return 0;
}

void drop_graphs(l2s_model* m) {
    for (auto& g : m->graphs) { (void)hipGraphExecDestroy(g.exec); (void)hipGraphDestroy(g.graph); }
    m->graphs.clear();
}

void free_model_device(l2s_model* m) {
    for (void* p : {(void*)m->blob, (void*)m->r_key, (void*)m->r_idx, m->r_tables, (void*)m->merge_scratch, m->lstm_planes, m->gemm_planes, m->unit_planes})
        if (p) (void)hipFree(p);
}

int pack_model(l2s_model* m, hipStream_t stream) {
    Packer P{m};
    if (pack_host(m, P)) return 1;
    if (m->opt.refresh_map && build_refresh_map(m, P, stream)) return 1;
    m->folded_valid = true;

    drop_graphs(m);
    if (m->blob) { (void)hipFree(m->blob); m->blob = nullptr; }
    m->blob_floats = (int64_t)P.blob.data.size();
    L2S_CHECK_HIP(hipMalloc(&m->blob, m->blob_floats * sizeof(float)));
    L2S_CHECK_HIP(hipMemcpyAsync(m->blob, P.blob.data.data(), m->blob_floats * sizeof(float), hipMemcpyHostToDevice, stream));
    L2S_CHECK_HIP(hipStreamSynchronize(stream));
    for (auto& f : P.fixups) *f.first = m->blob + f.second;
    m->finalized = true;
    m->has_enc = P.parts.enc;
    m->has_dec = P.parts.dec;
    m->has_spk = P.parts.spk;
    m->has_face = P.parts.face;
    return derive_all_planes(m, stream, true);
}

static int build_refresh_map(l2s_model* m, const Packer& P, hipStream_t stream) {
    std::vector<std::string> keys;
    for (auto& kv : m->host) keys.push_back(kv.first);
    std::sort(keys.begin(), keys.end());
    std::vector<int64_t> base(keys.size() + 1, 0);
    for (size_t i = 0; i < keys.size(); ++i) base[i + 1] = base[i] + (int64_t)m->host[keys[i]].size();
    L2S_REQUIRE(base.back() < 0x7F000000LL, "too many checkpoint elements for the refresh map");
    std::unordered_map<std::string, std::vector<float>> shadow;
    for (size_t i = 0; i < keys.size(); ++i) {
        std::vector<float> v(m->host[keys[i]].size());
        for (size_t j = 0; j < v.size(); ++j) { const uint32_t id = (uint32_t)(base[i] + (int64_t)j + 1); std::memcpy(&v[j], &id, 4); }
        shadow.emplace(keys[i], std::move(v));
    }
    Weights saved = m->w;
    m->host.swap(shadow);
    Packer P2{m};
    const int rc = pack_host(m, P2);
    m->host.swap(shadow);
    m->w = saved;
    if (rc) return 1;
    L2S_REQUIRE(P2.blob.data.size() == P.blob.data.size(), "refresh map: shadow pack differs in size");
    const int64_t n = (int64_t)P.blob.data.size();
    std::vector<int32_t> rk(n, -1), ri(n, 0);
    size_t cur = 0;
    for (int64_t i = 0; i < n; ++i) {
        uint32_t id; std::memcpy(&id, &P2.blob.data[i], 4);
        if (id == 0 || (int64_t)id > base.back()) continue;
        const int64_t g = (int64_t)id - 1;
        if (!(g >= base[cur] && g < base[cur + 1])) cur = (size_t)(std::upper_bound(base.begin(), base.end(), g) - base.begin()) - 1;
        const std::vector<float>& src = m->host[keys[cur]];
        const int64_t j = g - base[cur];
        uint32_t a, b; std::memcpy(&a, &P.blob.data[i], 4); std::memcpy(&b, &src[j], 4);
        if (a != b) continue;
        rk[i] = (int32_t)cur; ri[i] = (int32_t)j;
    }
    if (m->r_key) { (void)hipFree(m->r_key); m->r_key = nullptr; }
    if (m->r_idx) { (void)hipFree(m->r_idx); m->r_idx = nullptr; }
    L2S_CHECK_HIP(hipMalloc(&m->r_key, n * sizeof(int32_t)));
    L2S_CHECK_HIP(hipMalloc(&m->r_idx, n * sizeof(int32_t)));
    L2S_CHECK_HIP(hipMemcpyAsync(m->r_key, rk.data(), n * sizeof(int32_t), hipMemcpyHostToDevice, stream));
    L2S_CHECK_HIP(hipMemcpyAsync(m->r_idx, ri.data(), n * sizeof(int32_t), hipMemcpyHostToDevice, stream));
    L2S_CHECK_HIP(hipStreamSynchronize(stream));
    m->r_keys = keys;
    m->r_bn = P.bn_rec;
    m->r_sum = P.sum_rec;
    return 0;
}

struct RBn { const float *g, *b, *mu, *var, *bias; float *scale, *shift; int c; };
struct RSum { const float *a, *b; float* dst; int n, perm_H; };

__global__ __launch_bounds__(256) void refresh_gather_kernel(float* __restrict__ blob, const int32_t* __restrict__ rk, const int32_t* __restrict__ ri,
                                                             const float* const* __restrict__ ptrs, int64_t n) {
    for (int64_t i = (int64_t)blockIdx.x * 256 + threadIdx.x; i < n; i += (int64_t)gridDim.x * 256) {
        const int k = rk[i];
        if (k < 0) continue;
        const float* src = ptrs[k];
        if (src) blob[i] = src[ri[i]];
    }
}
__global__ __launch_bounds__(256) void refresh_bn_kernel(const RBn* __restrict__ recs) {
    const RBn r = recs[blockIdx.y];
    const int i = blockIdx.x * 256 + threadIdx.x;
    if (i >= r.c) return;
    bn_fold(r.g[i], r.b[i], r.mu[i], r.var[i], r.bias ? r.bias[i] : 0.f, BN_EPS, &r.scale[i], &r.shift[i]);
}
__global__ __launch_bounds__(256) void refresh_sum_kernel(const RSum* __restrict__ recs) {
    const RSum r = recs[blockIdx.y];
    const int np = blockIdx.x * 256 + threadIdx.x;
    if (np >= r.n) return;
    const int src = r.perm_H ? (np & 3) * r.perm_H + (np >> 2) : np;
    r.dst[np] = r.a[src] + r.b[src];
}

__global__ __launch_bounds__(256) void refresh_frontend_planes_kernel(const float* __restrict__ w, uint16_t* __restrict__ w3, uint16_t* __restrict__ w1) {
    const int idx = blockIdx.x * 256 + threadIdx.x;
    if (idx < FE_PLANE_ELEMS) fe_plane_fill(w, idx, w3, w1);
}

struct MergeSeg { const float* src; int ld, col0, k_lo, k_hi; };
__global__ __launch_bounds__(256) void merge_pack_kernel(float* __restrict__ dst, int N, int K, MergeSeg s0, MergeSeg s1, MergeSeg s2, int perm_H) {
    const int64_t total = (int64_t)N * K;
    for (int64_t idx = (int64_t)blockIdx.x * 256 + threadIdx.x; idx < total; idx += (int64_t)gridDim.x * 256) {
        const int k = idx % K, np = idx / K;
        const int r = perm_H ? (np & 3) * perm_H + (np >> 2) : np;
        const MergeSeg* segs[3] = {&s0, &s1, &s2};
        float v = 0.f;
#pragma unroll
        for (int q = 0; q < 3; ++q) {
            const MergeSeg& g = *segs[q];
            if (g.src && k >= g.k_lo && k < g.k_hi) v = g.src[(int64_t)r * g.ld + g.col0 + (k - g.k_lo)];
        }
        dst[frag16_index(np, k, K)] = v;
    }
}
__global__ __launch_bounds__(256) void merge_bias_kernel(float* __restrict__ out, int N, const float* __restrict__ a, const float* __restrict__ b,
                                                         const float* __restrict__ W, int ld, int col0, int K, const float* __restrict__ x, int perm_H) {
    const int np = blockIdx.x * 256 + threadIdx.x;
    if (np >= N) return;
    const int r = perm_H ? (np & 3) * perm_H + (np >> 2) : np;
    double acc = (double)a[r] + (b ? (double)b[r] : 0.0);
    for (int k = 0; k < K; ++k) acc += (double)W[(int64_t)r * ld + col0 + k] * (double)x[k];
    out[np] = (float)acc;
}
static int remerge_step_weights(l2s_model* m, hipStream_t s) {
    const std::string D = "decoder.";
    auto P = [&](const char* k) { return m->canon(D + k); };
    const float *wp1 = P("prenet.0.linear_layer.weight"), *bp1 = P("prenet.0.linear_layer.bias"), *wfc = P("fc_out.linear_layer.weight"), *bfc = P("fc_out.linear_layer.bias");
    const float *wih = P("decoder_rnn.weight_ih_l0"), *whh = P("decoder_rnn.weight_hh_l0"), *bih = P("decoder_rnn.bias_ih_l0"), *bhh = P("decoder_rnn.bias_hh_l0");
    const float *wap = P("attention_proj.linear_layer.weight"), *bap = P("attention_proj.linear_layer.bias");
    if (!(wp1 && bp1 && wfc && bfc && wih && whh && bih && bhh && wap && bap) || !m->w.pre1f.W || !m->w.lstm0f.W) return 0;
    if (!m->merge_scratch) L2S_CHECK_HIP(hipMalloc(&m->merge_scratch, sizeof(float) * ((int64_t)2048 * 512 + (int64_t)256 * 512)));
    float* prod_ap = m->merge_scratch; float* prod_p1 = prod_ap + (int64_t)2048 * 512;
    if (launch_gemm_bwd(bwd_dx(wih + 256, 512, wap, prod_ap, 512, 1, 2048, 2048, 256, 512, 1, 0, false), s, "train_merge_step_weights")) return 1;
    if (launch_gemm_bwd(bwd_dx(wp1, NM, wfc, prod_p1, 512, 1, 256, 256, NM, 512, 1, 0, false), s, "train_merge_step_weights")) return 1;
    ProfScope ps("train_merge_step_weights", s);
    const MergeSeg none{nullptr, 0, 0, 0, 0};
    hipLaunchKernelGGL(merge_pack_kernel, dim3(4096), dim3(256), 0, s, const_cast<float*>(m->w.lstm0f.W), 2048, 1536, MergeSeg{wih, 512, 0, 0, 512},
                       MergeSeg{prod_ap, 512, 0, 512, 1024}, MergeSeg{whh, 512, 0, 1024, 1536}, 512);
    hipLaunchKernelGGL(merge_pack_kernel, dim3(512), dim3(256), 0, s, const_cast<float*>(m->w.pre1f.W), 256, 512, MergeSeg{prod_p1, 512, 0, 0, 512}, none, none, 0);
    hipLaunchKernelGGL(merge_bias_kernel, dim3(8), dim3(256), 0, s, const_cast<float*>(m->w.lstm0f.bias), 2048, bih, bhh, wih, 512, 256, 256, bap, 512);
    hipLaunchKernelGGL(merge_bias_kernel, dim3(1), dim3(256), 0, s, const_cast<float*>(m->w.pre1f.bias), 256, bp1, (const float*)nullptr, wp1, NM, 0, NM, bfc, 0);
    L2S_CHECK_HIP(hipGetLastError());
    m->folded_valid = true;
    return 0;
}

int refresh_weights(l2s_model* m, hipStream_t s) {
    L2S_REQUIRE(m->finalized && m->r_key && m->r_idx, "no refresh map: set option refresh_map=1 before l2s_model_finalize");
    const size_t nk = m->r_keys.size(), nb = m->r_bn.size(), ns = m->r_sum.size();
    const size_t off_bn = align_up((int64_t)(nk * sizeof(float*)), 64), off_sum = off_bn + align_up((int64_t)(nb * sizeof(RBn)), 64);
    const size_t total = off_sum + ns * sizeof(RSum) + 64;
    m->r_tables_host.assign(total, 0);
    const float** ptrs = reinterpret_cast<const float**>(m->r_tables_host.data());
    for (size_t i = 0; i < nk; ++i) ptrs[i] = m->canon(m->r_keys[i]);
    RBn* bn = reinterpret_cast<RBn*>(m->r_tables_host.data() + off_bn);
    size_t nb_live = 0;
    int maxc = 1;
    for (const auto& r : m->r_bn) {
        RBn d{m->canon(r.p + ".weight"), m->canon(r.p + ".bias"), m->canon(r.p + ".running_mean"), m->canon(r.p + ".running_var"),
              r.bias_key.empty() ? nullptr : m->canon(r.bias_key), m->blob + r.so, m->blob + r.ho, r.c};
        if (!d.g && !d.b && !d.mu && !d.var) continue;
        L2S_REQUIRE(d.g && d.b && d.mu && d.var && (r.bias_key.empty() || d.bias), "refresh: BatchNorm tensors of a layer are only partly bound");
        bn[nb_live++] = d; maxc = std::max(maxc, r.c);
    }
    RSum* sm = reinterpret_cast<RSum*>(m->r_tables_host.data() + off_sum);
    size_t ns_live = 0;
    int maxn = 1;
    for (const auto& r : m->r_sum) {
        RSum d{m->canon(r.a), m->canon(r.b), m->blob + r.dst, r.n, r.perm_H};
        if (!d.a && !d.b) continue;
        L2S_REQUIRE(d.a && d.b, "refresh: bias pair only partly bound");
        sm[ns_live++] = d; maxn = std::max(maxn, r.n);
    }
    if ((int64_t)total > m->r_tables_bytes) {
        if (m->r_tables) (void)hipFree(m->r_tables);
        L2S_CHECK_HIP(hipMalloc(&m->r_tables, total));
        m->r_tables_bytes = (int64_t)total;
        m->r_tables_uploaded.clear();
    }
    if (m->r_tables_host != m->r_tables_uploaded) {
        L2S_CHECK_HIP(hipMemcpyAsync(m->r_tables, m->r_tables_host.data(), total, hipMemcpyHostToDevice, s));
        L2S_CHECK_HIP(hipStreamSynchronize(s));
        m->r_tables_uploaded = m->r_tables_host;
    }
    char* T = (char*)m->r_tables;
    {
        ProfScope ps("train_refresh_gather", s);
        hipLaunchKernelGGL(refresh_gather_kernel, dim3(4096), dim3(256), 0, s, m->blob, m->r_key, m->r_idx, reinterpret_cast<const float* const*>(T), m->blob_floats);
    }
    if (nb_live) hipLaunchKernelGGL(refresh_bn_kernel, dim3((maxc + 255) / 256, (unsigned)nb_live), dim3(256), 0, s, reinterpret_cast<const RBn*>(T + off_bn));
    if (ns_live) hipLaunchKernelGGL(refresh_sum_kernel, dim3((maxn + 255) / 256, (unsigned)ns_live), dim3(256), 0, s, reinterpret_cast<const RSum*>(T + off_sum));
    L2S_CHECK_HIP(hipGetLastError());
    if (const float* w3d = m->canon("encoder.frontend3D.0.weight"); w3d && m->w.fe.w3 && m->w.fe.w1) {
        ProfScope ps("train_refresh_frontend_planes", s);
        hipLaunchKernelGGL(refresh_frontend_planes_kernel, dim3(FE_PLANE_ELEMS / 256), dim3(256), 0, s, w3d,
                           reinterpret_cast<uint16_t*>(const_cast<float*>(m->w.fe.w3)), reinterpret_cast<uint16_t*>(const_cast<float*>(m->w.fe.w1)));
        L2S_CHECK_HIP(hipGetLastError());
    }
    if (derive_all_planes(m, s, false)) return 1;
    m->folded_valid = false;
    if (remerge_step_weights(m, s)) return 1;
    drop_graphs(m);
    return 0;
}

}
```

Measured before the change: 3.592 million mel-frames/s.

## Restructure two-frame front-end conv around row-granular weight planes and stepped slabs

Drops the x3p front-end kernel and sends both the pipelined and non-pipelined two-frame paths through a reworked x3q block. The reworked block is templated on a serial/overlapped schedule. A new row-granular weight layout (w3r) is packed on the host and refreshed on device, so the conv walks kernel rows in steps with zero-row padding instead of full 5-tap slabs. Weight and input staging is double-buffered per slab, and next-slab loads are interleaved into the MFMA loop. This is meant to skip MFMA work on padded taps and improve overlap, at the cost of more LDS (still capped for two blocks per CU), an extra weight copy in the blob, and more complex indexing.

Result: no change. 3.601 million mel-frames/s (median of 3 runs) (+0.3%).

```diff
diff --git a/lip2speech_amd/csrc/encoder_kernels.hip b/lip2speech_amd/csrc/encoder_kernels.hip
--- a/lip2speech_amd/csrc/encoder_kernels.hip
+++ b/lip2speech_amd/csrc/encoder_kernels.hip
@@ -370,256 +370,40 @@
     }
 }
 
-template <int HW>
-__global__ __launch_bounds__(256, 2) void frontend3d_x3p_kernel(const FrontendW w, const FrameSrc vsrc, int T, float* __restrict__ out) {
-    constexpr int H = HW, W = HW, Hc = H / 2, Wc = W / 2, Hp = Hc / 2, Wp = Wc / 2;
-    constexpr int P = FE_CR * Wc;
-    constexpr int PT = (P + 15) / 16;
-    constexpr int TPW = (PT + 3) / 4;
-    constexpr int XLD = 112, PLANE = FE_XROWS * XLD * 2;
-    static_assert(XLD >= W + 8 && (XLD / 2) % 32 == 24, "row pitch");
-    constexpr int XS = 3 * PLANE;
-    constexpr int WROW = 48, LROW = 32;
-    constexpr int WSP = 24 * LROW;
-    constexpr int WSO = 12 * WSP;
-    constexpr int WS = 2 * WSO;
-    constexpr int CS = P * (FE_CO / 2) * 4;
-    constexpr int SMEM = (XS + 2 * WS) > CS ? (XS + 2 * WS) : CS;
-    constexpr int NLD = ((FE_XROWS - 1) * (W / 4) + 255) / 256;
-    constexpr int NWU = WS / 16, NWC = NWU / 64;
-    static_assert(NWU % 64 == 0, "the weight operand is a whole number of wave-wide 16-byte pieces");
-    constexpr int SRC_SP = 32 * WROW / 16;
-    __shared__ __attribute__((aligned(16))) unsigned char smem[SMEM];
-    unsigned char* const Xs = smem;
-    unsigned char* const Ws0 = smem + XS;
-
-    const int NPAIR = (T + 1) / 2;
-    const int bg = blockIdx.y / NPAIR, t0 = 2 * (blockIdx.y - bg * NPAIR);
-    const bool has1 = t0 + 1 < T;
-    const int grp = bg / vsrc.per, b = bg - grp * vsrc.per;
-    const float* __restrict__ video = vsrc.p[grp];
-    const int p0 = blockIdx.x * FE_PR;
-    const int tid = threadIdx.x, wave = tid >> 6, lane = tid & 63;
-    const int li = lane & 15, kg = lane >> 4;
-    const int kr = ((kg & 1) << 1) | (kg >> 1);
-
-    for (int i = tid; i < XS / 16; i += 256) reinterpret_cast<uint4*>(Xs)[i] = make_uint4(0u, 0u, 0u, 0u);
-
-    int base[TPW];
-#pragma unroll
-    for (int j = 0; j < TPW; ++j) {
-        int p = (wave + 4 * j) * 16 + li;
-        p = p < P ? p : P - 1;
-        const int lr = p / Wc, c = p - lr * Wc;
-        base[j] = ((2 * lr + kr) * XLD + 2 * c) * 2;
-    }
-    int wof[3];
-#pragma unroll
-    for (int nt = 0; nt < 3; ++nt) {
-        const int q = nt * 16 + li, o = q >= FE_CO ? 1 : 0, ch = q - FE_CO * o;
-        wof[nt] = o * WSO + (kr >> 1) * (3 * WSP) + ch * LROW + (kr & 1) * 16;
-    }
-    f32x4 acc[TPW][3];
-#pragma unroll
-    for (int j = 0; j < TPW; ++j)
-#pragma unroll
-        for (int nt = 0; nt < 3; ++nt) acc[j][nt] = {0.f, 0.f, 0.f, 0.f};
-
-    const int gy0 = 4 * p0 - 5;
-    auto valid = [&](int sl) { const int d = sl % 6, tau = t0 - 2 + d; return tau >= 0 && tau < T && (d <= 4 || has1); };
-    auto next_valid = [&](int sl) { while (sl < 18 && !valid(sl)) ++sl; return sl; };
-
-    float4 rin[NLD];
-    auto fetch_piece = [&](int sl, int q) {
-        const int ci = sl / 6, d = sl - ci * 6;
-        const float* src = video + ((int64_t)(b * 3 + ci) * T + (t0 - 2 + d)) * (H * W);
-        const int i = tid + 256 * q;
-        const int row = i / (W / 4), x4 = i - row * (W / 4);
-        const int gy = gy0 + row;
-        rin[q] = make_float4(0.f, 0.f, 0.f, 0.f);
-        if (i < (FE_XROWS - 1) * (W / 4) && gy >= 0 && gy < H) rin[q] = *reinterpret_cast<const float4*>(src + gy * W + 4 * x4);
-    };
-    auto fetch = [&](int sl) {
-#pragma unroll
-        for (int q = 0; q < NLD; ++q) fetch_piece(sl, q);
-    };
-    auto dma_piece = [&](int sl, int buf, int kp) {
-        const int c = wave + 4 * kp;
-        if (c < NWC) {
-            const int ci = sl / 6, d = sl - ci * 6;
-            const uint4* w3 = reinterpret_cast<const uint4*>(w.w3);
-            unsigned char* const Wd = Ws0 + buf * WS;
-            const int i = c * 64 + lane;
-            const int o = i >= NWU / 2 ? 1 : 0, r = i - o * (NWU / 2);
-            const int sp = r / (WSP / 16), u = r - sp * (WSP / 16);
-            const int kt = d - o;
-            const bool on = kt >= 0 && kt <= 4 && (o == 0 || has1);
-            const uint4* src = on ? w3 + (int64_t)(ci * 5 + kt) * (12 * SRC_SP) + sp * SRC_SP + (u >> 1) * (WROW / 16) + (u & 1) : w3 + (24 * WROW) / 16;
-            __builtin_amdgcn_global_load_lds((const __attribute__((address_space(1))) void*)src,
-                                             (__attribute__((address_space(3))) void*)(Wd + c * 1024), 16, 0, 0);
-        }
-    };
-    constexpr int NDP = (NWC + 3) / 4;
-    auto dma_weights = [&](int sl, int buf) {
-#pragma unroll
-        for (int kp = 0; kp < NDP; ++kp) dma_piece(sl, buf, kp);
-    };
-    auto stage = [&]() {
-#pragma unroll
-        for (int q = 0; q < NLD; ++q) {
-            const int i = tid + 256 * q;
-            if (i < (FE_XROWS - 1) * (W / 4)) {
-                const int row = i / (W / 4), x4 = i - row * (W / 4);
-                unsigned char* dd = Xs + (row * XLD + 4 + 4 * x4) * 2;
-                uint2 hi, mid, lo;
-                fx_split4(rin[q], hi, mid, lo);
-                *reinterpret_cast<uint2*>(dd) = hi; *reinterpret_cast<uint2*>(dd + PLANE) = mid; *reinterpret_cast<uint2*>(dd + 2 * PLANE) = lo;
-            }
-        }
-    };
-
-    int sl = next_valid(0), nslab = 0;
-    if (sl < 18) { fetch(sl); dma_weights(sl, 0); }
-    while (sl < 18) {
-        __syncthreads();
-        stage();
-        const int d = sl % 6;
-        const bool on0 = d <= 4, on1 = d >= 1 && has1;
-        const int nxt = next_valid(sl + 1);
-        __syncthreads();
-        const bool more = nxt < 18;
-        static_assert(NDP + NLD <= 2 * TPW, "one request per pixel tile");
-        const unsigned char* const Ws = Ws0 + (nslab & 1) * WS;
-#pragma unroll
-        for (int S = 0; S < 2; ++S) {
-            fx_bf16x8 bh[3], bm[3], bl[3];
-#pragma unroll
-            for (int nt = 0; nt < 3; ++nt) {
-                const unsigned char* wp = Ws + wof[nt] + S * (2 * 3 * WSP);
-                bh[nt] = *reinterpret_cast<const fx_bf16x8*>(wp);
-                bm[nt] = *reinterpret_cast<const fx_bf16x8*>(wp + WSP);
-                bl[nt] = *reinterpret_cast<const fx_bf16x8*>(wp + 2 * WSP);
-            }
-#pragma unroll
-            for (int j = 0; j < TPW; ++j) {
-                if (more) {
-                    const int pos = S * TPW + j;
-                    if (pos < NDP) dma_piece(nxt, (nslab + 1) & 1, pos);
-                    else if (pos < NDP + NLD) fetch_piece(nxt, pos - NDP);
-                }
-                {
-                    const unsigned* ap = reinterpret_cast<const unsigned*>(Xs + base[j] + S * (4 * XLD * 2));
-                    const unsigned* am_ = reinterpret_cast<const unsigned*>(Xs + base[j] + S * (4 * XLD * 2) + PLANE);
-                    const unsigned* al_ = reinterpret_cast<const unsigned*>(Xs + base[j] + S * (4 * XLD * 2) + 2 * PLANE);
-                    const fx_bf16x8 ah = __builtin_bit_cast(fx_bf16x8, make_uint4(ap[0], ap[1], ap[2], ap[3]));
-                    const fx_bf16x8 am = __builtin_bit_cast(fx_bf16x8, make_uint4(am_[0], am_[1], am_[2], am_[3]));
-                    const fx_bf16x8 al = __builtin_bit_cast(fx_bf16x8, make_uint4(al_[0], al_[1], al_[2], al_[3]));
-#pragma unroll
-                    for (int nt = 0; nt < 3; ++nt) {
-                        if ((nt == 0 && !on0) || (nt == 2 && !on1)) continue;
-                        f32x4 a = acc[j][nt];
-                        a = __builtin_amdgcn_mfma_f32_16x16x32_bf16(al, bh[nt], a, 0, 0, 0);
-                        a = __builtin_amdgcn_mfma_f32_16x16x32_bf16(ah, bl[nt], a, 0, 0, 0);
-                        a = __builtin_amdgcn_mfma_f32_16x16x32_bf16(am, bm[nt], a, 0, 0, 0);
-                        a = __builtin_amdgcn_mfma_f32_16x16x32_bf16(am, bh[nt], a, 0, 0, 0);
-                        a = __builtin_amdgcn_mfma_f32_16x16x32_bf16(ah, bm[nt], a, 0, 0, 0);
-                        a = __builtin_amdgcn_mfma_f32_16x16x32_bf16(ah, bh[nt], a, 0, 0, 0);
-                        acc[j][nt] = a;
-                    }
-                }
-            }
-        }
-        sl = nxt; ++nslab;
-    }
-    __syncthreads();
-
-    float* Cs = reinterpret_cast<float*>(smem);
-    constexpr int CH = FE_CO / 2;
-    float sc[3], sh[3], slp[3];
-#pragma unroll
-    for (int nt = 0; nt < 3; ++nt) {
-        const int q = nt * 16 + li, ch = q >= FE_CO ? q - FE_CO : q;
-        sc[nt] = w.scale[ch]; sh[nt] = w.shift[ch]; slp[nt] = w.slope[ch];
-    }
-    for (int pass = 0; pass < (has1 ? 4 : 2); ++pass) {
-        const int o = pass >> 1, half = pass & 1;
-#pragma unroll
-        for (int nt = 0; nt < 3; ++nt) {
-            const int q = nt * 16 + li, qo = q >= FE_CO ? 1 : 0, ch = q - FE_CO * qo;
-            if (qo == o && ch >= half * CH && ch < (half + 1) * CH) {
-#pragma unroll
-                for (int j = 0; j < TPW; ++j) {
-                    if (wave + 4 * j < PT) {
-#pragma unroll
-                        for (int r = 0; r < 4; ++r) {
-                            const int p = (wave + 4 * j) * 16 + 4 * kg + r;
-                            if (p < P) {
-                                float v = acc[j][nt][r] * sc[nt] + sh[nt];
-                                v = v >= 0.f ? v : slp[nt] * v;
-                                Cs[p * CH + (ch - half * CH)] = v;
-                            }
-                        }
-                    }
-                }
-            }
-        }
-        __syncthreads();
-        const int f = bg * T + t0 + o;
-        for (int i = tid; i < FE_PR * Wp * CH; i += 256) {
-            const int ch = i % CH;
-            const int pw = (i / CH) % Wp;
-            const int prl = i / (CH * Wp);
-            const int pr = p0 + prl;
-            if (pr >= Hp) continue;
-            float m = -INFINITY;
-#pragma unroll
-            for (int dr = 0; dr < 3; ++dr) {
-                const int crow = 2 * pr - 1 + dr;
-                if (crow < 0 || crow >= Hc) continue;
-                const int lrow = 2 * prl + dr;
-#pragma unroll
-                for (int dc = -1; dc <= 1; ++dc) {
-                    const int cc = 2 * pw + dc;
-                    if (cc < 0 || cc >= Wc) continue;
-                    m = fmaxf(m, Cs[(lrow * Wc + cc) * CH + ch]);
-                }
-            }
-            out[(((int64_t)f * Hp + pr) * Wp + pw) * FE_CO + half * CH + ch] = m;
-        }
-        __syncthreads();
-    }
-}
-
-template <int HW>
+template <int HW, int SERIAL>
 __global__ __launch_bounds__(256, 2) void frontend3d_x3q_kernel(const FrontendW w, const FrameSrc vsrc, int T, float* __restrict__ out) {
     const int NPAIR = (T + 1) / 2;
     const int bg = blockIdx.y / NPAIR, t0 = 2 * (blockIdx.y - bg * NPAIR);
     const bool has1 = t0 + 1 < T;
     const int grp = bg / vsrc.per, b = bg - grp * vsrc.per;
     const float* __restrict__ video = vsrc.p[grp];
+#define FE_X3Q_SERIAL SERIAL
 #define FE_X3Q_PITCH T
 #define FE_X3Q_FRAME0 (bg * T)
 #include "frontend_x3q_block.inc"
 #undef FE_X3Q_PITCH
 #undef FE_X3Q_FRAME0
+#undef FE_X3Q_SERIAL
 }
 
 template <int HW>
 __global__ __launch_bounds__(256, 2) void frontend3d_x3q_ragged_kernel(const FrontendW w, const FrameSrc vsrc, const RaggedClip* __restrict__ clips,
                                                                        const int* __restrict__ pair_clip, float* __restrict__ out) {
-    const RaggedClip k = clips[pair_clip[blockIdx.y]];
-    const int T = k.len;
-    const int t0 = 2 * ((int)blockIdx.y - k.pair0);
+    const RaggedClip k_ = clips[pair_clip[blockIdx.y]];
+    const int T = k_.len;
+    const int t0 = 2 * ((int)blockIdx.y - k_.pair0);
     const bool has1 = t0 + 1 < T;
-    const int b = k.row;
+    const int b = k_.row;
     const float* __restrict__ video = vsrc.p[0];
 #pragma unroll
-    for (int g = 1; g < MAX_GROUP; ++g) video = k.g == g ? vsrc.p[g] : video;
-#define FE_X3Q_PITCH k.T
-#define FE_X3Q_FRAME0 k.frame0
+    for (int g = 1; g < MAX_GROUP; ++g) video = k_.g == g ? vsrc.p[g] : video;
+#define FE_X3Q_SERIAL 0
+#define FE_X3Q_PITCH k_.T
+#define FE_X3Q_FRAME0 k_.frame0
 #include "frontend_x3q_block.inc"
 #undef FE_X3Q_PITCH
 #undef FE_X3Q_FRAME0
+#undef FE_X3Q_SERIAL
 }
 
 int launch_frontend(const FrontendW& w, const FrameSrc& video, int B, int T, int H, int W, float* out, hipStream_t s, float* zout) {
@@ -635,12 +419,13 @@
         else hipLaunchKernelGGL((frontend3d_x3_kernel<88, 1>), grid, dim3(256), 0, s, w, video, T, out);
     } else if (!zout && w.w3 && w.pair) {
         dim3 gp((Hp + FE_PR - 1) / FE_PR, B * ((T + 1) / 2));
+        L2S_REQUIRE(w.w3r, "the two-frame front-end needs the row-granular weight planes");
         if (w.pipe) {
-            const unsigned pad = w.solo ? 4096u : 0u;
-            if (H == 96) hipLaunchKernelGGL((frontend3d_x3q_kernel<96>), gp, dim3(256), pad, s, w, video, T, out);
-            else hipLaunchKernelGGL((frontend3d_x3q_kernel<88>), gp, dim3(256), pad, s, w, video, T, out);
-        } else if (H == 96) hipLaunchKernelGGL((frontend3d_x3p_kernel<96>), gp, dim3(256), 0, s, w, video, T, out);
-        else hipLaunchKernelGGL((frontend3d_x3p_kernel<88>), gp, dim3(256), 0, s, w, video, T, out);
+            const unsigned pad = w.solo ? 8192u : 0u;
+            if (H == 96) hipLaunchKernelGGL((frontend3d_x3q_kernel<96, 0>), gp, dim3(256), pad, s, w, video, T, out);
+            else hipLaunchKernelGGL((frontend3d_x3q_kernel<88, 0>), gp, dim3(256), pad, s, w, video, T, out);
+        } else if (H == 96) hipLaunchKernelGGL((frontend3d_x3q_kernel<96, 1>), gp, dim3(256), 0, s, w, video, T, out);
+        else hipLaunchKernelGGL((frontend3d_x3q_kernel<88, 1>), gp, dim3(256), 0, s, w, video, T, out);
     } else if (!zout && w.w3) {
         if (H == 96) hipLaunchKernelGGL((frontend3d_x3_kernel<96, 3>), grid, dim3(256), 0, s, w, video, T, out);
         else hipLaunchKernelGGL((frontend3d_x3_kernel<88, 3>), grid, dim3(256), 0, s, w, video, T, out);
@@ -663,6 +448,7 @@
     dim3 gp((Hp + FE_PR - 1) / FE_PR, rg.NP);
     prof_count("frontend3d_ragged_pair_blocks", rg.NP);
     ProfScope ps("frontend3d_conv_bn_prelu_pool_ragged", s);
+    L2S_REQUIRE(w.w3r, "the two-frame front-end needs the row-granular weight planes");
     if (H == 96) hipLaunchKernelGGL((frontend3d_x3q_ragged_kernel<96>), gp, dim3(256), 0, s, w, video, rg.clips, rg.pair_clip, out);
     else hipLaunchKernelGGL((frontend3d_x3q_ragged_kernel<88>), gp, dim3(256), 0, s, w, video, rg.clips, rg.pair_clip, out);
     L2S_CHECK_HIP(hipGetLastError());
diff --git a/lip2speech_amd/csrc/frontend_x3q_block.inc b/lip2speech_amd/csrc/frontend_x3q_block.inc
--- a/lip2speech_amd/csrc/frontend_x3q_block.inc
+++ b/lip2speech_amd/csrc/frontend_x3q_block.inc
@@ -2,29 +2,29 @@
     constexpr int P = FE_CR * Wc;
     constexpr int PT = (P + 15) / 16;
     constexpr int TPW = (PT + 3) / 4;
-    constexpr int XLD = 112, PLANE = FE_XROWS * XLD * 2;
+    constexpr int NR = 2 * (FE_CR - 1) + 7;
+    constexpr int XLD = 112, PLANE = NR * XLD * 2;
     static_assert(XLD >= W + 8 && (XLD / 2) % 32 == 24, "row pitch");
     constexpr int XS = 3 * PLANE;
-    constexpr int WROW = 48, LROW = 32;
-    constexpr int WSP = 24 * LROW;
-    constexpr int WSO = 12 * WSP;
-    constexpr int WS = 2 * WSO;
+    constexpr int WSP = 48 * 16;
+    constexpr int WSR = 3 * WSP;
+    constexpr int WS = 7 * WSR;
+    constexpr int WSB = 16 * 1024;
+    constexpr int NWC = WSB / 1024, NDP = NWC / 4;
+    constexpr int XOFF = 2 * WSB, ZOFF = XOFF + 2 * XS;
     constexpr int CS = P * (FE_CO / 2) * 4;
-    constexpr int SMEM = (2 * XS + 2 * WS) > CS ? (2 * XS + 2 * WS) : CS;
-    constexpr int NLD = ((FE_XROWS - 1) * (W / 4) + 255) / 256;
-    constexpr int NWU = WS / 16, NWC = NWU / 64;
-    static_assert(NWU % 64 == 0, "the weight operand is a whole number of wave-wide 16-byte pieces");
-    constexpr int SRC_SP = 32 * WROW / 16;
+    constexpr int SMEM = (ZOFF + WSR) > CS ? (ZOFF + WSR) : CS;
+    static_assert(SMEM <= 80 * 1024, "two blocks per CU");
+    constexpr int NLD = (NR * (W / 4) + 255) / 256;
+    static_assert(NLD + NDP <= TPW, "one request per pixel tile of the step inside a slab");
     __shared__ __attribute__((aligned(16))) unsigned char smem[SMEM];
-    unsigned char* const Xs0 = smem;
-    unsigned char* const Ws0 = smem + 2 * XS;
 
     const int p0 = blockIdx.x * FE_PR;
     const int tid = threadIdx.x, wave = tid >> 6, lane = tid & 63;
     const int li = lane & 15, kg = lane >> 4;
     const int kr = ((kg & 1) << 1) | (kg >> 1);
 
-    for (int i = tid; i < 2 * XS / 16; i += 256) reinterpret_cast<uint4*>(Xs0)[i] = make_uint4(0u, 0u, 0u, 0u);
+    for (int i = tid; i < (2 * XS + WSR) / 16; i += 256) reinterpret_cast<uint4*>(smem + XOFF)[i] = make_uint4(0u, 0u, 0u, 0u);
 
     int base[TPW];
 #pragma unroll
@@ -32,13 +32,7 @@
         int p = (wave + 4 * j) * 16 + li;
         p = p < P ? p : P - 1;
         const int lr = p / Wc, c = p - lr * Wc;
-        base[j] = ((2 * lr + kr) * XLD + 2 * c) * 2;
-    }
-    int wof[3];
-#pragma unroll
-    for (int nt = 0; nt < 3; ++nt) {
-        const int q = nt * 16 + li, o = q >= FE_CO ? 1 : 0, ch = q - FE_CO * o;
-        wof[nt] = o * WSO + (kr >> 1) * (3 * WSP) + ch * LROW + (kr & 1) * 16;
+        base[j] = (2 * lr * XLD + 2 * c) * 2;
     }
     f32x4 acc[TPW][3];
 #pragma unroll
@@ -47,47 +41,36 @@
         for (int nt = 0; nt < 3; ++nt) acc[j][nt] = {0.f, 0.f, 0.f, 0.f};
 
     const int gy0 = 4 * p0 - 5;
-    auto valid = [&](int sl) { const int d = sl % 6, tau = t0 - 2 + d; return tau >= 0 && tau < T && (d <= 4 || has1); };
-    auto next_valid = [&](int sl) { while (sl < 18 && !valid(sl)) ++sl; return sl; };
+    const int dlo = t0 >= 2 ? 0 : 2 - t0;
+    const int dtop = has1 ? 5 : 4, dhi = T + 1 - t0 < dtop ? T + 1 - t0 : dtop;
+    const int nsl = 3 * (dhi - dlo + 1), nrows = 7 * nsl;
 
     float4 rin[NLD];
-    auto fetch_piece = [&](int sl, int q) {
-        const int ci = sl / 6, d = sl - ci * 6;
+    auto fetch_piece = [&](int k, int q) {
+        const int dk = k / 3, ci = k - 3 * dk, d = dlo + dk;
         const float* src = video + ((int64_t)(b * 3 + ci) * FE_X3Q_PITCH + (t0 - 2 + d)) * (H * W);
         const int i = tid + 256 * q;
         const int row = i / (W / 4), x4 = i - row * (W / 4);
         const int gy = gy0 + row;
         rin[q] = make_float4(0.f, 0.f, 0.f, 0.f);
-        if (i < (FE_XROWS - 1) * (W / 4) && gy >= 0 && gy < H) rin[q] = *reinterpret_cast<const float4*>(src + gy * W + 4 * x4);
+        if (i < NR * (W / 4) && gy >= 0 && gy < H) rin[q] = *reinterpret_cast<const float4*>(src + gy * W + 4 * x4);
     };
-    auto fetch = [&](int sl) {
-#pragma unroll
-        for (int q = 0; q < NLD; ++q) fetch_piece(sl, q);
-    };
-    auto dma_piece = [&](int sl, int buf, int kp) {
+    auto dma_piece = [&](int k, int kp) {
         const int c = wave + 4 * kp;
-        if (c < NWC) {
-            const int ci = sl / 6, d = sl - ci * 6;
-            const uint4* w3 = reinterpret_cast<const uint4*>(w.w3);
-            unsigned char* const Wd = Ws0 + buf * WS;
-            const int i = c * 64 + lane;
-            const int o = i >= NWU / 2 ? 1 : 0, r = i - o * (NWU / 2);
-            const int sp = r / (WSP / 16), u = r - sp * (WSP / 16);
-            const int kt = d - o;
-            const bool on = kt >= 0 && kt <= 4 && (o == 0 || has1);
-            const uint4* src = on ? w3 + (int64_t)(ci * 5 + kt) * (12 * SRC_SP) + sp * SRC_SP + (u >> 1) * (WROW / 16) + (u & 1) : w3 + (24 * WROW) / 16;
-            __builtin_amdgcn_global_load_lds((const __attribute__((address_space(1))) void*)src,
-                                             (__attribute__((address_space(3))) void*)(Wd + c * 1024), 16, 0, 0);
-        }
-    };
-    constexpr int NDP = (NWC + 3) / 4;
-    auto dma_weights = [&](int sl, int buf) {
-#pragma unroll
-        for (int kp = 0; kp < NDP; ++kp) dma_piece(sl, buf, kp);
+        const int dk = k / 3, ci = k - 3 * dk, d = dlo + dk;
+        const uint4* w3r = reinterpret_cast<const uint4*>(w.w3r);
+        const int i = c * 64 + lane;
+        const int rp = i / 48, q = i - 48 * rp;
+        const int o = q >= FE_CO ? 1 : 0, ch = q - FE_CO * o;
+        const int kt = d - o;
+        const bool on = i < WS / 16 && kt >= 0 && kt <= 4 && (o == 0 || has1);
+        const uint4* src = on ? w3r + ((int64_t)(ci * 5 + kt) * 21 + rp) * FE_CO + ch : reinterpret_cast<const uint4*>(w.w3) + (24 * 48) / 16;
+        __builtin_amdgcn_global_load_lds((const __attribute__((address_space(1))) void*)src,
+                                         (__attribute__((address_space(3))) void*)(smem + (k & 1) * WSB + c * 1024), 16, 0, 0);
     };
     auto stage_piece = [&](unsigned char* Xd, int q) {
         const int i = tid + 256 * q;
-        if (i < (FE_XROWS - 1) * (W / 4)) {
+        if (i < NR * (W / 4)) {
             const int row = i / (W / 4), x4 = i - row * (W / 4);
             unsigned char* dd = Xd + (row * XLD + 4 + 4 * x4) * 2;
             uint2 hi, mid, lo;
@@ -96,64 +79,71 @@
         }
     };
 
-    int sl = next_valid(0), nslab = 0;
-    if (sl < 18) {
-        fetch(sl); dma_weights(sl, 0);
-        __syncthreads();
-#pragma unroll
-        for (int q = 0; q < NLD; ++q) stage_piece(Xs0, q);
-    }
-    static_assert(NLD + NDP + NLD <= 2 * TPW, "one request / one staging piece per pixel tile");
-    while (sl < 18) {
-        __syncthreads();
-        const int d = sl % 6;
-        const bool on0 = d <= 4, on1 = d >= 1 && has1;
-        const int nxt = next_valid(sl + 1);
-        const bool more = nxt < 18;
-        const unsigned char* const Xs = Xs0 + (nslab & 1) * XS;
-        unsigned char* const Xn = Xs0 + ((nslab + 1) & 1) * XS;
-        const unsigned char* const Ws = Ws0 + (nslab & 1) * WS;
-#pragma unroll
-        for (int S = 0; S < 2; ++S) {
-            fx_bf16x8 bh[3], bm[3], bl[3];
-#pragma unroll
-            for (int nt = 0; nt < 3; ++nt) {
-                const unsigned char* wp = Ws + wof[nt] + S * (2 * 3 * WSP);
-                bh[nt] = *reinterpret_cast<const fx_bf16x8*>(wp);
-                bm[nt] = *reinterpret_cast<const fx_bf16x8*>(wp + WSP);
-                bl[nt] = *reinterpret_cast<const fx_bf16x8*>(wp + 2 * WSP);
-            }
-#pragma unroll
-            for (int j = 0; j < TPW; ++j) {
-                if (more) {
-                    const int pos = S * TPW + j;
-                    if (pos < NLD) fetch_piece(nxt, pos);
-                    else if (pos < NLD + NDP) dma_piece(nxt, (nslab + 1) & 1, pos - NLD);
-                    else if (pos >= 2 * TPW - NLD) stage_piece(Xn, pos - (2 * TPW - NLD));
+#pragma unroll
+    for (int q = 0; q < NLD; ++q) fetch_piece(0, q);
+#pragma unroll
+    for (int kp = 0; kp < NDP; ++kp) dma_piece(0, kp);
+    __syncthreads();
+#pragma unroll
+    for (int q = 0; q < NLD; ++q) stage_piece(smem + XOFF, q);
+    const int nsteps = (nrows + 3) >> 2;
+    for (int s = 0, kprev = -1; s < nsteps; ++s) {
+        const int klo = (4 * s) / 7, k = (4 * s + 3) / 7 < nsl ? (4 * s + 3) / 7 : nsl - 1;
+        const bool shared = klo != k, more = k + 1 < nsl && 4 * s + 4 <= nrows;
+        if (k != kprev) __syncthreads();
+        kprev = k;
+        const bool stage = more && !shared;
+        const bool fetch = more && (shared || !(k & 3));
+        const bool on0 = dlo + klo / 3 <= 4, on1 = has1 && dlo + k / 3 >= 1;
+        unsigned char* const Xn = smem + XOFF + ((k + 1) & 1) * XS;
+        if (FE_X3Q_SERIAL && stage) {
+#pragma unroll
+            for (int q = 0; q < NLD; ++q) fetch_piece(k + 1, q);
+#pragma unroll
+            for (int kp = 0; kp < NDP; ++kp) dma_piece(k + 1, kp);
+#pragma unroll
+            for (int q = 0; q < NLD; ++q) stage_piece(Xn, q);
+        }
+        const int g = 4 * s + kr, gc = g < nrows ? g : nrows - 1;
+        const int ks = gc / 7, r = gc - 7 * ks;
+        const unsigned char* const ax = smem + XOFF + (ks & 1) * XS + r * (XLD * 2);
+        const unsigned char* const wp = smem + (g < nrows ? (ks & 1) * WSB + r * WSR : ZOFF) + li * 16;
+        fx_bf16x8 bh[3], bm[3], bl[3];
+#pragma unroll
+        for (int nt = 0; nt < 3; ++nt) {
+            bh[nt] = *reinterpret_cast<const fx_bf16x8*>(wp + nt * 256);
+            bm[nt] = *reinterpret_cast<const fx_bf16x8*>(wp + nt * 256 + WSP);
+            bl[nt] = *reinterpret_cast<const fx_bf16x8*>(wp + nt * 256 + 2 * WSP);
+        }
+#pragma unroll
+        for (int j = 0; j < TPW; ++j) {
+            if (!FE_X3Q_SERIAL) {
+                if (j < NLD) { if (fetch) fetch_piece(k + 1, j); }
+                else if (j < NLD + NDP) { if (stage) dma_piece(k + 1, j - NLD); }
+                if (j >= TPW - NLD) { if (stage) stage_piece(Xn, j - (TPW - NLD)); }
+            }
+            {
+                const unsigned* ap = reinterpret_cast<const unsigned*>(ax + base[j]);
+                const unsigned* am_ = reinterpret_cast<const unsigned*>(ax + base[j] + PLANE);
+                const unsigned* al_ = reinterpret_cast<const unsigned*>(ax + base[j] + 2 * PLANE);
+                const fx_bf16x8 ah = __builtin_bit_cast(fx_bf16x8, make_uint4(ap[0], ap[1], ap[2], ap[3]));
+                const fx_bf16x8 am = __builtin_bit_cast(fx_bf16x8, make_uint4(am_[0], am_[1], am_[2], am_[3]));
+                const fx_bf16x8 al = __builtin_bit_cast(fx_bf16x8, make_uint4(al_[0], al_[1], al_[2], al_[3]));
+#pragma unroll
+                for (int nt = 0; nt < 3; ++nt) {
+                    if ((nt == 0 && !on0) || (nt == 2 && !on1)) continue;
+                    f32x4 a = acc[j][nt];
+                    a = __builtin_amdgcn_mfma_f32_16x16x32_bf16(al, bh[nt], a, 0, 0, 0);
+                    a = __builtin_amdgcn_mfma_f32_16x16x32_bf16(ah, bl[nt], a, 0, 0, 0);
+                    a = __builtin_amdgcn_mfma_f32_16x16x32_bf16(am, bm[nt], a, 0, 0, 0);
+                    a = __builtin_amdgcn_mfma_f32_16x16x32_bf16(am, bh[nt], a, 0, 0, 0);
+                    a = __builtin_amdgcn_mfma_f32_16x16x32_bf16(ah, bm[nt], a, 0, 0, 0);
+                    a = __builtin_amdgcn_mfma_f32_16x16x32_bf16(ah, bh[nt], a, 0, 0, 0);
+                    acc[j][nt] = a;
                 }
-                {
-                    const unsigned* ap = reinterpret_cast<const unsigned*>(Xs + base[j] + S * (4 * XLD * 2));
-                    const unsigned* am_ = reinterpret_cast<const unsigned*>(Xs + base[j] + S * (4 * XLD * 2) + PLANE);
-                    const unsigned* al_ = reinterpret_cast<const unsigned*>(Xs + base[j] + S * (4 * XLD * 2) + 2 * PLANE);
-                    const fx_bf16x8 ah = __builtin_bit_cast(fx_bf16x8, make_uint4(ap[0], ap[1], ap[2], ap[3]));
-                    const fx_bf16x8 am = __builtin_bit_cast(fx_bf16x8, make_uint4(am_[0], am_[1], am_[2], am_[3]));
-                    const fx_bf16x8 al = __builtin_bit_cast(fx_bf16x8, make_uint4(al_[0], al_[1], al_[2], al_[3]));
-#pragma unroll
-                    for (int nt = 0; nt < 3; ++nt) {
-                        if ((nt == 0 && !on0) || (nt == 2 && !on1)) continue;
-                        f32x4 a = acc[j][nt];
-                        a = __builtin_amdgcn_mfma_f32_16x16x32_bf16(al, bh[nt], a, 0, 0, 0);
-                        a = __builtin_amdgcn_mfma_f32_16x16x32_bf16(ah, bl[nt], a, 0, 0, 0);
-                        a = __builtin_amdgcn_mfma_f32_16x16x32_bf16(am, bm[nt], a, 0, 0, 0);
-                        a = __builtin_amdgcn_mfma_f32_16x16x32_bf16(am, bh[nt], a, 0, 0, 0);
-                        a = __builtin_amdgcn_mfma_f32_16x16x32_bf16(ah, bm[nt], a, 0, 0, 0);
-                        a = __builtin_amdgcn_mfma_f32_16x16x32_bf16(ah, bh[nt], a, 0, 0, 0);
-                        acc[j][nt] = a;
-                    }
-                }
-            }
-        }
-        sl = nxt; ++nslab;
+            }
+        }
+        if (shared && more) __syncthreads();
     }
     __syncthreads();
 
diff --git a/lip2speech_amd/csrc/l2s_common.h b/lip2speech_amd/csrc/l2s_common.h
--- a/lip2speech_amd/csrc/l2s_common.h
+++ b/lip2speech_amd/csrc/l2s_common.h
@@ -193,6 +193,7 @@
     int solo = 0;
     int pipe = 0;
     const float* w1;
+    const float* w3r = nullptr;
 };
 constexpr int MAX_GROUP = 8;
 struct FrameSrc { const float* p[MAX_GROUP]; int per; };
diff --git a/lip2speech_amd/csrc/l2s_pack.hip b/lip2speech_amd/csrc/l2s_pack.hip
--- a/lip2speech_amd/csrc/l2s_pack.hip
+++ b/lip2speech_amd/csrc/l2s_pack.hip
@@ -37,6 +37,12 @@
 __host__ __device__ inline void fe_plane_store(const FePlaneElem& e, int slab, int st, int n, int k, uint16_t* w3, uint16_t* w1) {
     for (int pl = 0; pl < 3; ++pl) w3[(int64_t)slab * FE_W3_SLAB + ((st * 3 + pl) * 32 + n) * 24 + k] = e.split[pl];
     w1[(int64_t)slab * FE_W1_SLAB + (st * 32 + n) * 24 + k] = e.rne;
+}
+constexpr int FE_ROW_ELEMS = 15 * 7 * 24 * 8, FE_W3R_U16 = 3 * FE_ROW_ELEMS;
+__host__ __device__ inline void fe_row_fill(const float* w, int idx, uint16_t* w3r) {
+    const int slot = idx & 7, n = (idx >> 3) % 24, r = (idx / 192) % 7, slab = idx / 1344;
+    const FePlaneElem e = fe_plane_elem(w, slab, r >> 1, n, 8 * (r & 1) + slot);
+    for (int pl = 0; pl < 3; ++pl) w3r[(((int64_t)(slab * 7 + r) * 3 + pl) * 24 + n) * 8 + slot] = e.split[pl];
 }
 __host__ __device__ inline void fe_plane_fill(const float* w, int idx, uint16_t* w3, uint16_t* w1) {
     const int k = idx & 15, n = (idx >> 4) & 31, st = (idx >> 9) & 3, slab = idx >> 11;
@@ -154,6 +160,11 @@
             std::memcpy(&P.blob.data[o1], w1.data(), w1.size() * 2);
             P.bind(&w.fe.w3, o3);
             P.bind(&w.fe.w1, o1);
+            const int64_t o3r = P.blob.alloc(FE_W3R_U16 / 2);
+            std::vector<uint16_t> w3r(FE_W3R_U16, 0);
+            for (int idx = 0; idx < FE_ROW_ELEMS; ++idx) fe_row_fill(v->data(), idx, w3r.data());
+            std::memcpy(&P.blob.data[o3r], w3r.data(), w3r.size() * 2);
+            P.bind(&w.fe.w3r, o3r);
         }
         P.bn(E + "frontend3D.1", 24, nullptr, &w.fe.scale, &w.fe.shift);
         P.copy(E + "frontend3D.2.weight", 24, &w.fe.slope);
@@ -716,9 +727,12 @@
     r.dst[np] = r.a[src] + r.b[src];
 }
 
-__global__ __launch_bounds__(256) void refresh_frontend_planes_kernel(const float* __restrict__ w, uint16_t* __restrict__ w3, uint16_t* __restrict__ w1) {
+static_assert(FE_ROW_ELEMS <= FE_PLANE_ELEMS, "one grid refreshes both arrays");
+__global__ __launch_bounds__(256) void refresh_frontend_planes_kernel(const float* __restrict__ w, uint16_t* __restrict__ w3, uint16_t* __restrict__ w1,
+                                                                      uint16_t* __restrict__ w3r) {
     const int idx = blockIdx.x * 256 + threadIdx.x;
     if (idx < FE_PLANE_ELEMS) fe_plane_fill(w, idx, w3, w1);
+    if (idx < FE_ROW_ELEMS) fe_row_fill(w, idx, w3r);
 }
 
 struct MergeSeg { const float* src; int ld, col0, k_lo, k_hi; };
@@ -815,10 +829,11 @@
     if (nb_live) hipLaunchKernelGGL(refresh_bn_kernel, dim3((maxc + 255) / 256, (unsigned)nb_live), dim3(256), 0, s, reinterpret_cast<const RBn*>(T + off_bn));
     if (ns_live) hipLaunchKernelGGL(refresh_sum_kernel, dim3((maxn + 255) / 256, (unsigned)ns_live), dim3(256), 0, s, reinterpret_cast<const RSum*>(T + off_sum));
     L2S_CHECK_HIP(hipGetLastError());
-    if (const float* w3d = m->canon("encoder.frontend3D.0.weight"); w3d && m->w.fe.w3 && m->w.fe.w1) {
+    if (const float* w3d = m->canon("encoder.frontend3D.0.weight"); w3d && m->w.fe.w3 && m->w.fe.w1 && m->w.fe.w3r) {
         ProfScope ps("train_refresh_frontend_planes", s);
         hipLaunchKernelGGL(refresh_frontend_planes_kernel, dim3(FE_PLANE_ELEMS / 256), dim3(256), 0, s, w3d,
-                           reinterpret_cast<uint16_t*>(const_cast<float*>(m->w.fe.w3)), reinterpret_cast<uint16_t*>(const_cast<float*>(m->w.fe.w1)));
+                           reinterpret_cast<uint16_t*>(const_cast<float*>(m->w.fe.w3)), reinterpret_cast<uint16_t*>(const_cast<float*>(m->w.fe.w1)),
+                           reinterpret_cast<uint16_t*>(const_cast<float*>(m->w.fe.w3r)));
         L2S_CHECK_HIP(hipGetLastError());
     }
     if (derive_all_planes(m, s, false)) return 1;
```
